# ishine/TTS-3

Hardware: AMD Instinct MI355X
Metric: audio samples/sec + RTF, HiFiGAN-v1 22.05kHz 80-mel, batch 32 @ 1/2/4/8 GPU (higher is better)
Workload: dtype fp32 (power-of-2 scaled fp16 hi/lo split on fp16 MFMA, fp32 accumulate); 1 GPU; HiFiGAN-v1 22.05kHz inference, [32,80,1024] mel per GPU (replicate pad 5), fp32; model=HiFiGAN-v1 (hifigan_config.py generator_model_params), global_batch=32, seq_len=1024, parallelism=dp1 (utterance sharding; no collectives)

## Files before the change

tts-3_amd/csrc/common.hpp:

```cpp
#pragma once

#include <hip/hip_runtime.h>

#include <cstdint>
#include <stdexcept>
#include <string>

namespace tts {

struct Error : std::runtime_error {
  int code;
  Error(int c, const std::string& m) : std::runtime_error(m), code(c) {}
};

#define TTS_HIP_CHECK(expr)                                                               \
  do {                                                                                    \
    hipError_t _e = (expr);                                                               \
    if (_e != hipSuccess)                                                                 \
      throw ::tts::Error(2, std::string(#expr) + " failed: " + hipGetErrorString(_e));    \
  } while (0)

#define TTS_REQUIRE(cond, code, msg)                    \
  do {                                                  \
    if (!(cond)) throw ::tts::Error((code), (msg));     \
  } while (0)

typedef float f32x4 __attribute__((ext_vector_type(4)));
typedef float f32x16 __attribute__((ext_vector_type(16)));

__device__ __forceinline__ float lrelu(float x, float slope) { return x > 0.f ? x : x * slope; }

constexpr int kPlaneXB16 = 1;
constexpr int kPlaneYB16 = 2;

struct Conv1dArgs {
  const float* x;
  const float* w;
  const float* bias;
  const float* res;
  float* y;
  float* z;
  const float* cvec;
  const float* mask;
  int64_t x_bstride;
  int Cin, Cout, Tin, Tout;
  int dil, pad, rep_pad;
  int n_chunks;
  float in_slope, out_slope;
  int zmode;
  float zdiv;
  const unsigned* amax_in;
  unsigned* amax_out;
  int w_exp;
  int ups;
  int64_t o_bstride;
  int64_t cvec_bstride;
  int mask_res;
  int wn_rows;
  int gate;
  int planes;
};

constexpr int kSplitGateTile = 20;
constexpr int kSplitWinoTile = 21;
bool wino_supported(int mode, int Cout, int Cin, int K, int dil);
bool wino_enabled();
void launch_wino(int mode, const Conv1dArgs& a, int B, int K, hipStream_t s);
inline int gate_row_order(int rho, int H) {
  const int j = rho / 128, r = rho % 128;
  return r < 64 ? 64 * j + r : H + 64 * j + (r - 64);
}

struct ResPairArgs {
  Conv1dArgs c1;
  Conv1dArgs c2;
  const float* post_w;
  float post_bias;
  float post_slope;
  float* wav;
};
bool resblock_pair_supported(int mode, int C, int K, int dil);
bool resblock_pair_preferred(int mode, int C, int K, int dil);
bool resblock_pair128(int mode, int C, int K);
void launch_resblock_pair(int mode, const ResPairArgs& a, int B, int K, int C, hipStream_t s);

struct ResBlock3Args {
  const float* x;
  const unsigned* amax_in;
  const float* w[6];
  const float* bias[6];
  int w_exp[6];
  int dil[3];
  float* z;
  int zmode;
  float zdiv;
  unsigned* amax_out;
  int T;
  int planes;
  const float* up_w;
  const float* up_bias;
  int up_w_exp;
  float* up_y;
  unsigned* up_amax;
  const float* zp[2];
  int nzp;
};
bool resblock3_supported(int mode, int C, int K, const int* dil);
bool resblock3_up_supported(int mode, int C, int K, const int* dil);
void launch_resblock3(int mode, const ResBlock3Args& a, int B, int C, int K, hipStream_t s);
bool resblock2_supported(int mode, int C, int K, const int* dil);
bool resblock2_preferred(int mode, int C, int K, const int* dil);
int resblock2_geo64(int mode);
void launch_resblock2(int mode, const ResBlock3Args& a, int B, int C, int K, int geo64, hipStream_t s);

struct ConvTile {
  int BM, BN, TM, TN, CK;
  int PD = 1;
  int WINO = 0;
};

struct ConvTArgs {
  const float* x;
  const float* w;
  const float* bias;
  float* y;
  int Cin, Cout, Tin;
  int n_chunks;
  float in_slope;
  unsigned* amax_out;
  const float* cvec;
};

struct PostArgs {
  const float* z;
  const float* w;
  float bias;
  float* y;
  int Cin, T;
  float in_slope;
  int z_b16;
};

int conv1d_tile_for(int Cout, int K, int Cin, int dil, bool res);
ConvTile conv1d_tile(int idx);
int conv1d_num_tiles();
void launch_conv1d(const Conv1dArgs& a, int B, int K, int tile_idx, hipStream_t s);
int convT_tile_for(int Cout, int U);
ConvTile convT_tile(int idx, int U);
void launch_convT(const ConvTArgs& a, int B, int U, int tile_idx, hipStream_t s);
void launch_conv_post(const PostArgs& a, int B, hipStream_t s);
void launch_mel_window(const float* mel, int B, int C, int T, int pad, int64_t w0, int W, float* out, hipStream_t s);
void launch_cond_vec(const float* g, const float* Wc, const float* bc, float* cvec, int B, int Cc,
                     int C0, hipStream_t s);

constexpr int MATH_FP32 = 0;
constexpr int MATH_FP32_X6 = 1;
constexpr int MATH_FP32_F16X3 = 2;
constexpr int MATH_BF16 = 3;
constexpr int MATH_LAST = MATH_BF16;

ConvTile conv1d_split_tile(int mode, int idx);
int conv1d_split_num_tiles(int mode);
int conv1d_split_tile_for(int mode, int Cout, int K, int Cin, int dil, bool res);
void launch_conv1d_split(int mode, const Conv1dArgs& a, int B, int K, int tile_idx, hipStream_t s);
bool convT_res_supported(int mode, const Conv1dArgs& a);
void launch_convT_res(int mode, const Conv1dArgs& a, int B, hipStream_t s);
void launch_amax(const float* x, int64_t n, int B, unsigned* slots, hipStream_t s, int64_t stride = 0);

inline bool is_split_mode(int mode) { return mode == MATH_FP32_X6 || mode == MATH_FP32_F16X3 || mode == MATH_BF16; }
inline ConvTile conv_tile(int mode, int idx) {
  return is_split_mode(mode) ? conv1d_split_tile(mode, idx) : conv1d_tile(idx);
}
inline int conv_tile_for(int mode, int Cout, int K, int Cin, int dil, bool res) {
  return is_split_mode(mode) ? conv1d_split_tile_for(mode, Cout, K, Cin, dil, res)
                             : conv1d_tile_for(Cout, K, Cin, dil, res);
}
inline int conv_num_tiles(int mode) { return is_split_mode(mode) ? conv1d_split_num_tiles(mode) : conv1d_num_tiles(); }
inline void launch_conv(int mode, const Conv1dArgs& a, int B, int K, int tile, hipStream_t s) {
  if (is_split_mode(mode)) launch_conv1d_split(mode, a, B, K, tile, s);
  else launch_conv1d(a, B, K, tile, s);
}

void pack_conv1d(const float* w, int Cout, int Cin, int K, const ConvTile& t, float* out);
int64_t packed_conv1d_numel(int Cout, int Cin, int K, const ConvTile& t);
void pack_convT(const float* w, int Cin, int Cout, int U, const ConvTile& t, float* out);
int64_t packed_convT_numel(int Cin, int Cout, int U, const ConvTile& t);
__host__ __device__ constexpr int quad_pos(int q) { return q == 1 ? 2 : (q == 2 ? 1 : q); }
int pack_conv1d_split(int mode, const float* w, int Cout, int Cin, int K, const ConvTile& t, float* out,
                      bool quad_perm = true);
int64_t packed_conv1d_split_numel(int mode, int Cout, int Cin, int K, const ConvTile& t);
int pack_convT_split(int mode, const float* w, int Cin, int Cout, int U, const ConvTile& t, float* out);
int pack_conv1d_wino(int mode, const float* w, int Cout, int Cin, int K, const ConvTile& t, float* out);
inline int64_t packed_conv_numel(int mode, int Cout, int Cin, int K, const ConvTile& t) {
  if (t.WINO) return packed_conv1d_split_numel(mode, Cout, Cin, 7 * ((K + 3) / 4), t);
  return is_split_mode(mode) ? packed_conv1d_split_numel(mode, Cout, Cin, K, t) : packed_conv1d_numel(Cout, Cin, K, t);
}
inline int pack_conv(int mode, const float* w, int Cout, int Cin, int K, const ConvTile& t, float* out) {
  if (t.WINO) return pack_conv1d_wino(mode, w, Cout, Cin, K, t, out);
  if (is_split_mode(mode)) return pack_conv1d_split(mode, w, Cout, Cin, K, t, out);
  pack_conv1d(w, Cout, Cin, K, t, out);
  return 0;
}

inline int ceil_div(int a, int b) { return (a + b - 1) / b; }

}
```

tts-3_amd/csrc/hifigan.cpp:

```cpp
#include "hifigan.hpp"

#include <algorithm>
#include <cmath>
#include <cstdlib>
#include <vector>

namespace tts {

namespace {
bool valid_conv_k(int k) { return k == 1 || k == 3 || k == 5 || k == 7 || k == 11; }
}

std::vector<int64_t> hifigan_weight_shapes(const TtsHifiganCfg& c) {
  std::vector<int64_t> n;
  const int C0 = c.upsample_initial_channel;
  n.push_back((int64_t)C0 * c.in_channels * 7);
  n.push_back(C0);
  for (int i = 0; i < c.num_upsamples; ++i) {
    const int ci = C0 >> i, co = C0 >> (i + 1);
    n.push_back((int64_t)ci * co * c.upsample_kernel_sizes[i]);
    n.push_back(co);
  }
  for (int i = 0; i < c.num_upsamples; ++i) {
    const int ch = C0 >> (i + 1);
    for (int j = 0; j < c.num_kernels; ++j) {
      const int k = c.resblock_kernel_sizes[j];
      const int nconv = (c.resblock_type == 1) ? 6 : 2;
      for (int m = 0; m < nconv; ++m) {
        n.push_back((int64_t)ch * ch * k);
        n.push_back(ch);
      }
    }
  }
  const int cl = C0 >> c.num_upsamples;
  n.push_back((int64_t)c.out_channels * cl * 7);
  if (c.conv_post_bias) n.push_back(c.out_channels);
  if (c.cond_channels > 0) {
    n.push_back((int64_t)C0 * c.cond_channels);
    n.push_back(C0);
  }
  if (c.cond_in_each_up_layer) {
    for (int i = 0; i < c.num_upsamples; ++i) {
      n.push_back((int64_t)(C0 >> (i + 1)) * c.cond_channels);
      n.push_back(C0 >> (i + 1));
    }
  }
  return n;
}

void hifigan_validate(const TtsHifiganCfg& c) {
  TTS_REQUIRE(c.in_channels >= 1, 1, "in_channels must be >= 1");
  TTS_REQUIRE(c.out_channels == 1, 3, "only out_channels == 1 is implemented");
  TTS_REQUIRE(c.resblock_type == 1 || c.resblock_type == 2, 1, "resblock_type must be '1' or '2'");
  TTS_REQUIRE(c.num_kernels >= 1 && c.num_kernels <= TTS_MAX_KERNELS, 1, "bad num_kernels");
  TTS_REQUIRE(c.num_upsamples >= 1 && c.num_upsamples <= TTS_MAX_UPSAMPLES, 1, "bad num_upsamples");
  const int need_d = c.resblock_type == 1 ? 3 : 2;
  TTS_REQUIRE(c.num_dilations >= need_d && c.num_dilations <= TTS_MAX_DILATIONS, 1,
              "resblock_dilation_sizes too short for the resblock type");
  for (int j = 0; j < c.num_kernels; ++j) {
    TTS_REQUIRE(valid_conv_k(c.resblock_kernel_sizes[j]), 3,
                "resblock kernel size " + std::to_string(c.resblock_kernel_sizes[j]) +
                    " not implemented (1,3,5,7,11)");
    for (int m = 0; m < need_d; ++m) {
      const int d = c.resblock_dilation_sizes[j][m];
      TTS_REQUIRE(d >= 1 && (c.resblock_kernel_sizes[j] - 1) * d <= 96, 3,
                  "resblock (kernel_size-1)*dilation must be <= 96");
    }
  }
  int C = c.upsample_initial_channel;
  for (int i = 0; i < c.num_upsamples; ++i) {
    const int u = c.upsample_factors[i];
    TTS_REQUIRE(u == 2 || u == 4 || u == 8, 3, "upsample factor must be 2, 4 or 8");
    TTS_REQUIRE(c.upsample_kernel_sizes[i] == 2 * u, 3,
                "upsample kernel size must equal 2*factor (polyphase kernel)");
    C >>= 1;
    TTS_REQUIRE(C >= 1, 1, "upsample_initial_channel too small for the number of upsamples");
  }
  TTS_REQUIRE(c.inference_padding >= 0, 1, "inference_padding must be >= 0");
  TTS_REQUIRE(c.cond_channels >= 0, 1, "cond_channels must be >= 0");
  TTS_REQUIRE(!c.cond_in_each_up_layer || c.cond_channels > 0, 1, "cond_in_each_up_layer needs cond_channels > 0");
  TTS_REQUIRE(c.math_mode >= MATH_FP32 && c.math_mode <= MATH_LAST, 1, "unknown math_mode");
}

Hifigan::Hifigan(const TtsHifiganCfg& cfg, const float* const* hw, int device)
    : cfg_(cfg), device_(device) {
  hifigan_validate(cfg_);
  DeviceGuard g(device_);
  const auto shapes = hifigan_weight_shapes(cfg_);
  for (size_t i = 0; i < shapes.size(); ++i)
    TTS_REQUIRE(hw[i] != nullptr, 1, "weight pointer " + std::to_string(i) + " is NULL");

  const int C0 = cfg_.upsample_initial_channel;
  const int mode = cfg_.math_mode;
  const char* nf = std::getenv("TTS_MI355X_NO_PAIR_FUSION");
  const bool pair_fusion = !(nf && nf[0] == '1');
  const char* pf = std::getenv("TTS_MI355X_POST_FUSION");
  post_fusion_ = !(pf && pf[0] == '0');
  const char* ms = std::getenv("TTS_MI355X_MRF_STREAMS");
  nbs_ = ms ? std::max(1, std::min(std::atoi(ms), cfg.num_kernels)) : cfg.num_kernels;
  nbs_env_ = ms != nullptr;
  const char* sb = std::getenv("TTS_MI355X_SUBBATCH");
  n_lanes_ = sb ? std::max(1, std::min(std::atoi(sb), 8)) : 2;
  rb2_geo64_ = resblock2_geo64(mode);
  const char* bp = std::getenv("TTS_MI355X_BF16_PLANES");
  planes16_ = mode == MATH_BF16 && !(bp && bp[0] == '0') && cfg_.num_upsamples >= 1 &&
              cfg_.upsample_factors[0] % 8 == 0;
  size_t wi = 0;
  std::vector<std::pair<const float*, const float*>> src;
  auto add_conv = [&](int Cin, int Cout, int K, int dil, const char* fam, bool res, int lmode, bool pair128 = false) {
    ConvLayer L;
    L.Cin = Cin; L.Cout = Cout; L.K = K; L.dil = dil; L.pad = dil * (K - 1) / 2;
    L.mode = lmode;
    L.tile = conv_tile_for(lmode, Cout, K, Cin, dil, res);
    if (pair128) {
      L.tile = 7;
      L.name = std::string(fam) + "_k" + std::to_string(K) + "_c" + std::to_string(Cout);
      return L;
    }
    const bool wino_k3 = [] {
      const char* e = std::getenv("TTS_MI355X_WINO_K3");
      return e && e[0] == '1';
    }();
    const bool k_ok = K >= 7 || (K == 3 && Cout >= 256 && wino_k3);
    if (std::string(fam) == "mrf_conv" && k_ok && wino_enabled() && wino_supported(lmode, Cout, Cin, K, dil)) {
      L.tile = kSplitWinoTile;
      fam = "mrf_wino";
    }
    L.name = std::string(fam) + "_k" + std::to_string(K) + "_c" + std::to_string(Cout);
    return L;
  };

  pre_ = add_conv(cfg_.in_channels, C0, 7, 1, "conv_pre", false, mode);
  src.push_back({hw[wi], hw[wi + 1]}); wi += 2;
  for (int i = 0; i < cfg_.num_upsamples; ++i) {
    ConvTLayer L;
    L.Cin = C0 >> i; L.Cout = C0 >> (i + 1); L.U = cfg_.upsample_factors[i];
    L.mode = mode;
    L.tile = is_split_mode(mode) ? conv_tile_for(mode, L.U * L.Cout, 2, L.Cin, 1, false) : convT_tile_for(L.Cout, L.U);
    L.name = "ups_u" + std::to_string(L.U) + "_c" + std::to_string(L.Cout);
    ups_.push_back(L);
  }
  std::vector<std::pair<const float*, const float*>> usrc;
  for (int i = 0; i < cfg_.num_upsamples; ++i) { usrc.push_back({hw[wi], hw[wi + 1]}); wi += 2; }

  for (int i = 0; i < cfg_.num_upsamples; ++i) {
    const int ch = C0 >> (i + 1);
    for (int j = 0; j < cfg_.num_kernels; ++j) {
      const int k = cfg_.resblock_kernel_sizes[j];
      ResBlock rb;
      if (cfg_.resblock_type == 1) {
        const float* w1[3]; const float* b1[3]; const float* w2[3]; const float* b2[3];
        for (int m = 0; m < 3; ++m) { w1[m] = hw[wi]; b1[m] = hw[wi + 1]; wi += 2; }
        for (int m = 0; m < 3; ++m) { w2[m] = hw[wi]; b2[m] = hw[wi + 1]; wi += 2; }
        rb.fused = pair_fusion;
        const bool p128 = pair_fusion && resblock_pair128(mode, ch, k);
        bool tiles_ok = true;
        for (int m = 0; m < 3; ++m) {
          rb.convs.push_back(add_conv(ch, ch, k, cfg_.resblock_dilation_sizes[j][m], "mrf_conv", false, mode, p128));
          src.push_back({w1[m], b1[m]});
          rb.convs.push_back(add_conv(ch, ch, k, 1, "mrf_conv", true, mode, p128));
          src.push_back({w2[m], b2[m]});
          for (int c = 0; c < 2; ++c) {
            const ConvTile t = conv_tile(mode, rb.convs[2 * m + c].tile);
            const int dil = rb.convs[2 * m].dil;
            tiles_ok = tiles_ok && !t.WINO && t.CK % 16 == 0 && ch % t.CK == 0 && ch % t.BM == 0;
            rb.fused = rb.fused && !t.WINO && t.CK == 16 && ceil_div(ch, t.BM) * t.BM == ch &&
                       resblock_pair_preferred(mode, ch, k, dil);
          }
        }
        rb.fused3 = pair_fusion && tiles_ok;
      } else {
        bool tiles_ok = true;
        for (int m = 0; m < 2; ++m) {
          rb.convs.push_back(add_conv(ch, ch, k, cfg_.resblock_dilation_sizes[j][m], "mrf_conv", true, mode));
          src.push_back({hw[wi], hw[wi + 1]}); wi += 2;
          const ConvTile t = conv_tile(mode, rb.convs[m].tile);
          tiles_ok = tiles_ok && !t.WINO && t.CK % 16 == 0 && ch % t.CK == 0 && ch % t.BM == 0;
        }
        rb.fused2 = pair_fusion && tiles_ok;
      }
      if (rb.fused2 || (cfg_.resblock_type == 1 && rb.fused3)) {
        const int policy = [] {
          const char* e = std::getenv("TTS_MI355X_RESBLOCK3");
          if (!e) return 1 << 30;
          if (std::string(e) == "all") return 1 << 30;
          return std::atoi(e);
        }();
        const std::string wk = [] {
          const char* e = std::getenv("TTS_MI355X_RB1_WHOLE_K");
          return std::string(e ? e : "");
        }();
        const bool k_ok = k == 3 || wk.find(std::to_string(k)) != std::string::npos;
        if (cfg_.resblock_type == 1)
          rb.fused3 = ch <= policy && k_ok && resblock3_supported(mode, ch, k, cfg_.resblock_dilation_sizes[j]);
        else
          rb.fused2 = ch <= policy && resblock2_preferred(mode, ch, k, cfg_.resblock_dilation_sizes[j]);
      }
      res_.push_back(rb);
    }
  }
  ups_fused_.assign(cfg_.num_upsamples, 0);
  const char* uf = std::getenv("TTS_MI355X_UPS_FUSION");
  if (!(uf && uf[0] == '0') && cfg_.resblock_type == 1 && cfg_.num_kernels <= 3 && !cfg_.cond_in_each_up_layer &&
      !planes16_) {
    for (int i = 0; i + 1 < cfg_.num_upsamples; ++i) {
      const int ch = C0 >> (i + 1);
      const ConvTLayer& u = ups_[i + 1];
      if (!res_[i * cfg_.num_kernels].fused3 || u.U != 2 || !is_split_mode(u.mode)) continue;
      const ConvTile t = conv_tile(u.mode, u.tile);
      const bool tile_ok = !t.WINO && t.CK % 16 == 0 && ch % t.CK == 0 && ch % t.BM == 0;
      ups_fused_[i] = tile_ok && resblock3_up_supported(mode, ch, cfg_.resblock_kernel_sizes[0],
                                                        cfg_.resblock_dilation_sizes[0]);
    }
  }
  const float* post_w = hw[wi]; wi += 1;
  post_bias_ = cfg_.conv_post_bias ? hw[wi][0] : 0.f;
  if (cfg_.conv_post_bias) wi += 1;

  HostArena arena;
  std::vector<ConvLayer*> convs;
  convs.push_back(&pre_);
  for (auto& rb : res_) for (auto& c : rb.convs) convs.push_back(&c);
  for (size_t i = 0; i < convs.size(); ++i) {
    ConvLayer& c = *convs[i];
    arena.put_conv(c, c.mode, conv_tile(c.mode, c.tile), src[i].first, src[i].second);
  }
  for (size_t i = 0; i < ups_.size(); ++i) {
    auto& u = ups_[i];
    if (is_split_mode(u.mode)) {
      const ConvTile t = conv_tile(u.mode, u.tile);
      u.n_chunks = ceil_div(u.Cin, t.CK);
      const size_t o = arena.alloc(packed_conv_numel(u.mode, u.U * u.Cout, u.Cin, 2, t), &u.w);
      u.w_exp = pack_convT_split(u.mode, usrc[i].first, u.Cin, u.Cout, u.U, t, arena.at(o));
      std::vector<float> bias((size_t)u.U * u.Cout);
      for (int co = 0; co < u.Cout; ++co)
        for (int ph = 0; ph < u.U; ++ph) bias[(size_t)co * u.U + ph] = usrc[i].second[co];
      arena.put_bias(bias.data(), u.U * u.Cout, t, &u.b);
    } else {
      const ConvTile t = convT_tile(u.tile, u.U);
      u.n_chunks = ceil_div(u.Cin, t.CK);
      const size_t o = arena.alloc(packed_convT_numel(u.Cin, u.Cout, u.U, t), &u.w);
      pack_convT(usrc[i].first, u.Cin, u.Cout, u.U, t, arena.at(o));
      arena.put_bias(usrc[i].second, u.Cout, t, &u.b);
    }
  }
  arena.put(post_w, (size_t)(C0 >> cfg_.num_upsamples) * 7, &post_wd_);
  if (cfg_.cond_channels > 0) {
    arena.put(hw[wi], (size_t)C0 * cfg_.cond_channels, &cond_wd_);
    arena.put(hw[wi + 1], C0, &cond_bd_);
    wi += 2;
  }
  if (cfg_.cond_in_each_up_layer) {
    up_cond_.resize(cfg_.num_upsamples);
    for (int i = 0; i < cfg_.num_upsamples; ++i) {
      const size_t ci = C0 >> (i + 1);
      arena.put(hw[wi], ci * cfg_.cond_channels, &up_cond_[i].first);
      arena.put(hw[wi + 1], ci, &up_cond_[i].second);
      wi += 2;
    }
  }
  arena.upload(device_, arena_);
  hop_ = 1;
  for (int i = 0; i < cfg_.num_upsamples; ++i) hop_ *= cfg_.upsample_factors[i];
}

Hifigan::~Hifigan() {
  DeviceGuard g(device_);
  for (Lane& ln : lanes_) {
    for (hipStream_t st : ln.branch) (void)hipStreamDestroy(st);
    if (ln.own) (void)hipStreamDestroy(ln.own);
    for (hipEvent_t e : ln.ev_z) (void)hipEventDestroy(e);
    if (ln.ev_ups) (void)hipEventDestroy(ln.ev_ups);
    if (ln.ev_done) (void)hipEventDestroy(ln.ev_done);
  }
  if (ev_start_) (void)hipEventDestroy(ev_start_);
}

int64_t Hifigan::out_len(int T, int pad) const { return (int64_t)hop_ * (T + 2 * pad); }

int64_t Hifigan::plane_floats(int B, int T, int pad) const {
  const int64_t L = T + 2 * pad;
  int64_t best = (int64_t)cfg_.upsample_initial_channel * L;
  int64_t len = L;
  for (int i = 0; i < cfg_.num_upsamples; ++i) {
    len *= cfg_.upsample_factors[i];
    const int64_t c = (int64_t)(cfg_.upsample_initial_channel >> (i + 1)) * len;
    if (c > best) best = c;
  }
  return ((best * B + 63) / 64) * 64;
}

int Hifigan::n_planes(int nbs) const { return 2 + 2 * nbs; }

int Hifigan::split_nbs() const { return nbs_env_ ? nbs_ : 1; }

void Hifigan::ensure_lanes() {
  if (!lanes_.empty()) return;
  auto stream = [] {
    hipStream_t st;
    TTS_HIP_CHECK(hipStreamCreateWithFlags(&st, hipStreamNonBlocking));
    return st;
  };
  auto event = [] {
    hipEvent_t e;
    TTS_HIP_CHECK(hipEventCreateWithFlags(&e, hipEventDisableTiming));
    return e;
  };
  lanes_.resize(n_lanes_);
  for (int i = 0; i < n_lanes_; ++i) {
    Lane& ln = lanes_[i];
    if (i > 0) ln.own = stream();
    for (int j = 1; j < nbs_; ++j) ln.branch.push_back(stream());
    ln.ev_ups = event();
    ln.ev_done = event();
    for (int j = 0; j < cfg_.num_kernels; ++j) ln.ev_z.push_back(event());
  }
  ev_start_ = event();
}

int64_t Hifigan::lane_bytes(int B, int64_t L, int nbs) const {
  const int64_t cond = cond_floats(B);
  const int64_t amax = cfg_.math_mode == MATH_FP32_F16X3 ? (int64_t)amax_groups() * B * 64 : 0;
  return ((n_planes(nbs) * plane_floats(B, (int)L, 0) + cond + amax + 63) / 64 * 64) * (int64_t)sizeof(float);
}

int Hifigan::amax_groups() const { return 2 + cfg_.num_upsamples * (2 + cfg_.num_kernels * 6); }
int Hifigan::stage_group(int i) const { return 2 + i * (2 + cfg_.num_kernels * 6); }

int64_t Hifigan::cond_floats(int B) const {
  if (cfg_.cond_channels <= 0) return 0;
  int64_t n = (((int64_t)B * cfg_.upsample_initial_channel + 63) / 64) * 64;
  if (cfg_.cond_in_each_up_layer)
    for (int i = 0; i < cfg_.num_upsamples; ++i)
      n += (((int64_t)B * (cfg_.upsample_initial_channel >> (i + 1)) + 63) / 64) * 64;
  return n;
}

int Hifigan::window_halo() const {
  double r = 3.0, rate = 1.0;
  for (int i = 0; i < cfg_.num_upsamples; ++i) {
    r += 1.5 / rate;
    rate *= cfg_.upsample_factors[i];
    int widest = 0;
    for (int j = 0; j < cfg_.num_kernels; ++j) {
      const int h = (cfg_.resblock_kernel_sizes[j] - 1) / 2;
      int w = 0;
      for (int m = 0; m < (cfg_.resblock_type == 1 ? 3 : 2); ++m)
        w += h * cfg_.resblock_dilation_sizes[j][m] + (cfg_.resblock_type == 1 ? h : 0);
      widest = std::max(widest, w);
    }
    r += widest / rate;
  }
  r += 3.0 / rate;
  return (int)std::ceil(r) + 2;
}

int64_t Hifigan::max_window_frames() const {
  int64_t cr = cfg_.upsample_initial_channel, rate = 1;
  for (int i = 0; i < cfg_.num_upsamples; ++i) {
    rate *= cfg_.upsample_factors[i];
    cr = std::max(cr, (int64_t)(cfg_.upsample_initial_channel >> (i + 1)) * rate);
  }
  return ((int64_t(1) << 29) - 1) / cr;
}

int64_t Hifigan::window_payload() const {
  const char* e = std::getenv("TTS_MI355X_WINDOW_FRAMES");
  const int64_t cap = max_window_frames() - 2 * window_halo();
  if (e && std::atoll(e) > 0) return std::min<int64_t>(std::atoll(e), cap);
  return cap;
}

bool Hifigan::windowed(int64_t L) const {
  const char* e = std::getenv("TTS_MI355X_WINDOW_FRAMES");
  return L > max_window_frames() || (e && std::atoll(e) > 0 && L > std::atoll(e));
}

int64_t Hifigan::plain_workspace_bytes(int B, int64_t L, bool window) const {
  const int nl = std::min(n_lanes_, B);
  if (window || nl == 1) return lane_bytes(B, L, nbs_);
  int64_t lanes = 0;
  for (int i = 0; i < nl; ++i) lanes += lane_bytes(lane_batch(B, i), L, split_nbs());
  return std::max(lane_bytes(B, L, 1), lanes);
}

int64_t Hifigan::window_buffer_bytes(int B, int64_t W) const {
  return ((((int64_t)B * cfg_.in_channels * W + 63) / 64) * 64 + (int64_t)B * hop_ * W) * (int64_t)sizeof(float);
}

int64_t Hifigan::workspace_bytes(int B, int T, int pad) const {
  const int64_t L = (int64_t)T + 2 * pad;
  if (!windowed(L)) return plain_workspace_bytes(B, L, false);
  const int64_t W = std::min<int64_t>(L, window_payload() + 2 * window_halo());
  return plain_workspace_bytes(B, W, true) + window_buffer_bytes(B, W);
}

void Hifigan::reserve_plain(int B, int64_t L, bool window) {
  const int64_t need = plain_workspace_bytes(B, L, window);
  ws_.grow(device_, (size_t)need, "workspace");
}

void Hifigan::reserve(int B, int T, int pad) {
  const int64_t L = (int64_t)T + 2 * pad;
  if (!windowed(L)) {
    reserve_plain(B, L);
    return;
  }
  const int64_t W = std::min<int64_t>(L, window_payload() + 2 * window_halo());
  reserve_plain(B, W, true);
  win_.grow(device_, (size_t)window_buffer_bytes(B, W), "window buffers");
}

void Hifigan::forward(const float* mel, int B, int C, int T, int pad, const float* gvec, float* wav,
                      hipStream_t s, Profiler* prof) {
  TTS_REQUIRE(mel && wav, 1, "NULL input/output pointer");
  TTS_REQUIRE(B >= 1, 1, "batch must be >= 1");
  TTS_REQUIRE(C == cfg_.in_channels, 1,
              "mel has " + std::to_string(C) + " channels, generator expects " + std::to_string(cfg_.in_channels));
  TTS_REQUIRE(T >= 1, 1, "T must be >= 1");
  TTS_REQUIRE(pad >= 0, 1, "pad must be >= 0");
  TTS_REQUIRE(cfg_.cond_channels == 0 || gvec != nullptr, 1, "cond_channels > 0 requires g");
  const int64_t L = (int64_t)T + 2 * pad;
  if (!windowed(L)) {
    DeviceGuard dg(device_);
    reserve_plain(B, L);
    if (prof) {
      forward_plain(mel, B, C, T, pad, gvec, wav, s, prof, ws_.as<>(), nullptr);
      return;
    }
    ensure_lanes();
    const int nl = std::min(n_lanes_, B);
    for (Lane& ln : lanes_) ln.nbs = nl > 1 ? split_nbs() : nbs_;
    if (nl == 1) {
      forward_plain(mel, B, C, T, pad, gvec, wav, s, nullptr, ws_.as<>(), &lanes_[0]);
      return;
    }
    TTS_HIP_CHECK(hipEventRecord(ev_start_, s));
    float* ws = ws_.as<>();
    int b0 = 0;
    for (int i = 0; i < nl; ++i) {
      const int Bi = lane_batch(B, i);
      Lane& ln = lanes_[i];
      const hipStream_t si = i == 0 ? s : ln.own;
      if (i > 0) TTS_HIP_CHECK(hipStreamWaitEvent(si, ev_start_, 0));
      forward_plain(mel + (int64_t)b0 * C * T, Bi, C, T, pad,
                    gvec ? gvec + (int64_t)b0 * cfg_.cond_channels : nullptr, wav + (int64_t)b0 * out_len(T, pad), si,
                    nullptr, ws, &ln);
      if (i > 0) {
        TTS_HIP_CHECK(hipEventRecord(ln.ev_done, si));
        TTS_HIP_CHECK(hipStreamWaitEvent(s, ln.ev_done, 0));
      }
      ws += lane_bytes(Bi, L, ln.nbs) / (int64_t)sizeof(float);
      b0 += Bi;
    }
    return;
  }
  DeviceGuard dg(device_);
  reserve(B, T, pad);
  const int h = window_halo();
  const int64_t P = window_payload();
  TTS_REQUIRE(P >= 1, 3, "window payload must be >= 1 frame");
  const int64_t Wmax = std::min<int64_t>(L, P + 2 * h);
  float* melw = win_.as<>();
  float* outw = melw + (((int64_t)B * C * Wmax + 63) / 64) * 64;
  for (int64_t s0 = 0; s0 < L; s0 += P) {
    const int64_t s1 = std::min(L, s0 + P);
    const int64_t w0 = std::max<int64_t>(0, s0 - h), w1 = std::min(L, s1 + h);
    const int W = (int)(w1 - w0);
    run(prof, s, "mel_window", 0.0, 8.0 * B * C * (double)W,
        [&] { launch_mel_window(mel, B, C, T, pad, w0, W, melw, s); });
    if (!prof) {
      ensure_lanes();
      lanes_[0].nbs = nbs_;
    }
    forward_plain(melw, B, C, W, 0, gvec, outw, s, prof, ws_.as<>(), prof ? nullptr : &lanes_[0]);
    TTS_HIP_CHECK(hipMemcpy2DAsync(wav + hop_ * s0, sizeof(float) * hop_ * L, outw + hop_ * (s0 - w0),
                                   sizeof(float) * hop_ * W, sizeof(float) * hop_ * (s1 - s0), B,
                                   hipMemcpyDeviceToDevice, s));
  }
}

void Hifigan::forward_plain(const float* mel, int B, int C, int T, int pad, const float* gvec, float* wav,
                            hipStream_t s, Profiler* prof, float* ws, Lane* lane) {
  DeviceGuard g(device_);

  const int64_t plane = plane_floats(B, T, pad);
  float* bufZ = ws;
  float* bufO = ws + plane;
  float* bufT0 = ws + 3 * plane;
  const int np = n_planes(lane ? lane->nbs : 1);
  float* cvec = cfg_.cond_channels > 0 ? ws + np * plane : nullptr;
  const bool h3 = cfg_.math_mode == MATH_FP32_F16X3;
  unsigned* amax = h3 ? reinterpret_cast<unsigned*>(ws + np * plane + cond_floats(B)) : nullptr;
  const int nbs = lane ? lane->nbs : 1;
  const bool conc = nbs > 1;
  const int K = cfg_.num_kernels;
  auto bstream = [&](int j) { return std::max(0, j - (K - nbs)); };
  auto slots = [&](int grp) -> unsigned* { return amax ? amax + (size_t)grp * B * 64 : nullptr; };
  if (h3) TTS_HIP_CHECK(hipMemsetAsync(amax, 0, (size_t)amax_groups() * B * 64 * sizeof(unsigned), s));

  const int L = T + 2 * pad;
  const int C0 = cfg_.upsample_initial_channel;
  bool post_done = false;
  if (cvec) {
    run(prof, s, "cond_layer", 2.0 * B * C0 * cfg_.cond_channels, 4.0 * (B * cfg_.cond_channels + C0 * cfg_.cond_channels + B * C0),
        [&] { launch_cond_vec(gvec, cond_wd_, cond_bd_, cvec, B, cfg_.cond_channels, C0, s); });
  }

  auto conv = [&](const ConvLayer& Ld, const float* x, int Tin, int Tout, int rep, float in_slope,
                  float out_slope, const float* res, float* y, int zmode, const float* cv,
                  const unsigned* amax_in = nullptr, unsigned* amax_out = nullptr, hipStream_t st = nullptr) {
    if (!st) st = s;
    Conv1dArgs a{};
    a.amax_in = amax_in; a.amax_out = amax_out; a.w_exp = Ld.w_exp;
    a.x = x; a.w = Ld.w; a.bias = Ld.b; a.res = res; a.y = y; a.z = bufZ; a.cvec = cv;
    a.Cin = Ld.Cin; a.Cout = Ld.Cout; a.Tin = Tin; a.Tout = Tout;
    a.dil = Ld.dil; a.pad = Ld.pad; a.rep_pad = rep; a.n_chunks = Ld.n_chunks;
    a.in_slope = in_slope; a.out_slope = out_slope; a.zmode = zmode; a.zdiv = (float)cfg_.num_kernels;
    a.planes = planes16_ ? (x == mel ? kPlaneYB16 : kPlaneXB16 | kPlaneYB16) : 0;
    const double ex = (planes16_ && x != mel) ? 2.0 : 4.0, ey = planes16_ ? 2.0 : 4.0;
    const double flops = 2.0 * B * Ld.Cout * (double)Ld.Cin * Ld.K * Tout;
    double bytes = ex * B * Ld.Cin * Tin + 4.0 * Ld.Cout * Ld.Cin * Ld.K + ey * B * Ld.Cout * Tout;
    if (res) bytes += ey * B * Ld.Cout * (double)Tout;
    if (zmode >= 2) bytes += ey * B * Ld.Cout * (double)Tout;
    run(prof, st, Ld.name.c_str(), flops, bytes, [&] { launch_conv(Ld.mode, a, B, Ld.K, Ld.tile, st); });
  };

  if (h3)
    run(prof, s, "amax_mel", 0.0, 4.0 * B * C * (double)T,
        [&] { launch_amax(mel, (int64_t)C * T, B, slots(0), s); });
  conv(pre_, mel, T, L, pad, 1.f, 1.f, nullptr, bufZ, 0, cvec, slots(0), slots(1));

  int len = L;
  const float* cur = bufZ;
  float* upvec = cvec ? cvec + (((int64_t)B * C0 + 63) / 64) * 64 : nullptr;
  for (int i = 0; i < cfg_.num_upsamples; ++i) {
    const ConvTLayer& U = ups_[i];
    const int g0 = stage_group(i);
    const float* ucv = nullptr;
    if (cfg_.cond_in_each_up_layer) {
      const int ci = U.Cout;
      run(prof, s, "cond_up", 2.0 * B * ci * cfg_.cond_channels, 4.0 * (B * cfg_.cond_channels + ci * cfg_.cond_channels + B * ci),
          [&] { launch_cond_vec(gvec, up_cond_[i].first, up_cond_[i].second, upvec, B, cfg_.cond_channels, ci, s); });
      ucv = upvec;
      upvec += (((int64_t)B * ci + 63) / 64) * 64;
    }
    const unsigned* z_amax = slots(i == 0 ? 1 : stage_group(i - 1) + 1 + cfg_.num_kernels * 6);
    const int lout = len * U.U;
    const double uflops = 2.0 * B * U.Cout * (double)U.Cin * 2 * lout;
    const double es = planes16_ ? 2.0 : 4.0;
    const double ubytes = es * ((double)B * U.Cin * len + (double)B * U.Cout * lout) + 4.0 * U.Cin * U.Cout * 2 * U.U;
    const bool fuse = ups_fused_[i] != 0;
    const bool ups_done = i > 0 && ups_fused_[i - 1] != 0;
    if (ups_done) {
    } else if (is_split_mode(U.mode)) {
      Conv1dArgs a{};
      a.planes = planes16_ ? kPlaneXB16 | kPlaneYB16 : 0;
      a.x = cur; a.w = U.w; a.bias = U.b; a.y = bufO;
      a.Cin = U.Cin; a.Cout = U.U * U.Cout; a.Tin = len; a.Tout = len + 1;
      a.dil = 1; a.pad = 1; a.n_chunks = U.n_chunks;
      a.in_slope = 0.1f; a.out_slope = 1.f; a.zdiv = 1.f;
      a.amax_in = z_amax; a.amax_out = slots(g0); a.w_exp = U.w_exp; a.ups = U.U;
      a.cvec = ucv;
      run(prof, s, U.name.c_str(), uflops, ubytes, [&] { launch_conv(U.mode, a, B, 2, U.tile, s); });
    } else {
      ConvTArgs ta{};
      ta.x = cur; ta.w = U.w; ta.bias = U.b; ta.y = bufO;
      ta.Cin = U.Cin; ta.Cout = U.Cout; ta.Tin = len; ta.n_chunks = U.n_chunks; ta.in_slope = 0.1f;
      ta.cvec = ucv;
      run(prof, s, U.name.c_str(), uflops, ubytes, [&] { launch_convT(ta, B, U.U, U.tile, s); });
    }
    len = lout;
    if (conc) TTS_HIP_CHECK(hipEventRecord(lane->ev_ups, s));
    float* rplane[TTS_MAX_KERNELS] = {};
    for (int jj = 0; jj < K; ++jj) {
      const int j = fuse ? (jj + 1) % K : jj;
      const ResBlock& rb = res_[i * K + j];
      const int bj = conc ? bstream(j) : 0;
      const hipStream_t sj = bj > 0 ? lane->branch[bj - 1] : s;
      float* bufX = ws + (2 + 2 * bj) * plane;
      float* bufT = bj == 0 ? bufT0 : bufX + plane;
      if (bj > 0) TTS_HIP_CHECK(hipStreamWaitEvent(sj, lane->ev_ups, 0));
      float* const xres = (fuse && j + 1 < K && (conc ? bstream(j + 1) : 0) == bj) ? bufZ : bufX;
      rplane[j] = xres;
      auto zorder = [&] {
        if (!fuse && bj > 0 && bstream(j - 1) != bj) TTS_HIP_CHECK(hipStreamWaitEvent(sj, lane->ev_z[j - 1], 0));
      };
      auto zdone = [&] {
        if (conc) TTS_HIP_CHECK(hipEventRecord(lane->ev_z[j], sj));
      };
      const int zlast = fuse ? 0 : ((cfg_.num_kernels == 1 || j == 0) ? 1 : (j == cfg_.num_kernels - 1 ? 3 : 2));
      const int gj = g0 + 1 + j * 6;
      const int gz = g0 + 1 + cfg_.num_kernels * 6;
      if (fuse && j == 0) {
        const ConvTLayer& Un = ups_[i + 1];
        ResBlock3Args ra{};
        ra.x = bufO; ra.amax_in = slots(g0);
        for (int c = 0; c < 6; ++c) { ra.w[c] = rb.convs[c].w; ra.bias[c] = rb.convs[c].b; ra.w_exp[c] = rb.convs[c].w_exp; }
        for (int m = 0; m < 3; ++m) ra.dil[m] = rb.convs[2 * m].dil;
        ra.zdiv = (float)K;
        ra.T = len;
        ra.nzp = K - 1;
        for (int p = 1; p < K; ++p) {
          ra.zp[p - 1] = rplane[p];
          if (conc && bstream(p) > 0) TTS_HIP_CHECK(hipStreamWaitEvent(s, lane->ev_z[p], 0));
        }
        ra.up_w = Un.w; ra.up_bias = Un.b; ra.up_w_exp = Un.w_exp;
        ra.up_y = bufT0; ra.up_amax = slots(stage_group(i + 1));
        const ConvLayer& L1 = rb.convs[0];
        const double flops = 12.0 * B * L1.Cout * (double)L1.Cin * L1.K * len +
                             2.0 * B * Un.Cout * (double)Un.Cin * 2 * (2.0 * len);
        const double bytes = 4.0 * B * L1.Cout * (double)len * (K + 1) + 4.0 * 6.0 * L1.Cout * L1.Cin * L1.K +
                             4.0 * Un.Cin * Un.Cout * 2 * Un.U;
        const std::string nm = "mrf_block_k" + std::to_string(L1.K) + "_c" + std::to_string(L1.Cout);
        run(prof, s, nm.c_str(), flops, bytes, [&] { launch_resblock3(L1.mode, ra, B, L1.Cout, L1.K, s); });
        std::swap(bufO, bufT0);
      } else if (cfg_.resblock_type == 1 && rb.fused3) {
        ResBlock3Args ra{};
        ra.x = bufO; ra.amax_in = slots(g0);
        ra.planes = planes16_ ? kPlaneXB16 | kPlaneYB16 : 0;
        for (int c = 0; c < 6; ++c) { ra.w[c] = rb.convs[c].w; ra.bias[c] = rb.convs[c].b; ra.w_exp[c] = rb.convs[c].w_exp; }
        for (int m = 0; m < 3; ++m) ra.dil[m] = rb.convs[2 * m].dil;
        ra.z = fuse ? xres : bufZ; ra.zmode = fuse ? 1 : zlast; ra.zdiv = (float)cfg_.num_kernels;
        ra.amax_out = !fuse && j == cfg_.num_kernels - 1 ? slots(gz) : nullptr;
        ra.T = len;
        const ConvLayer& L1 = rb.convs[0];
        const double flops = 12.0 * B * L1.Cout * (double)L1.Cin * L1.K * len;
        const double bytes = (planes16_ ? 2.0 : 4.0) * B * L1.Cout * len * (zlast >= 2 ? 3 : 2) +
                             4.0 * 6.0 * L1.Cout * L1.Cin * L1.K;
        const std::string nm = "mrf_block_k" + std::to_string(L1.K) + "_c" + std::to_string(L1.Cout);
        zorder();
        run(prof, sj, nm.c_str(), flops, bytes, [&] { launch_resblock3(L1.mode, ra, B, L1.Cout, L1.K, sj); });
        zdone();
      } else if (cfg_.resblock_type == 1 && rb.fused) {
        for (int m = 0; m < 3; ++m) {
          const ConvLayer& L1 = rb.convs[2 * m];
          const ConvLayer& L2 = rb.convs[2 * m + 1];
          const float* xin = (m == 0) ? bufO : (m == 1 ? bufX : bufT);
          const bool last = (m == 2);
          float* xout = (m == 1) ? bufT : (last ? xres : bufX);
          ResPairArgs pa{};
          Conv1dArgs& c1 = pa.c1;
          c1.x = xin; c1.w = L1.w; c1.bias = L1.b; c1.Cin = L1.Cin; c1.Cout = L1.Cout; c1.Tin = len; c1.Tout = len;
          c1.dil = L1.dil; c1.pad = L1.pad; c1.n_chunks = L1.n_chunks; c1.in_slope = 0.1f; c1.out_slope = 0.1f;
          c1.zdiv = 1.f; c1.w_exp = L1.w_exp;
          c1.planes = planes16_ ? kPlaneXB16 | kPlaneYB16 : 0;
          c1.amax_in = (m == 0) ? slots(g0) : slots(gj + 2 * m - 1);
          Conv1dArgs& c2 = pa.c2;
          c2.x = nullptr; c2.w = L2.w; c2.bias = L2.b; c2.res = xin; c2.y = xout; c2.z = bufZ;
          c2.Cin = L2.Cin; c2.Cout = L2.Cout; c2.Tin = len; c2.Tout = len; c2.dil = 1; c2.pad = L2.pad;
          c2.n_chunks = L2.n_chunks; c2.in_slope = 1.f; c2.out_slope = 1.f; c2.zmode = last ? zlast : 0;
          c2.zdiv = (float)cfg_.num_kernels; c2.w_exp = L2.w_exp;
          c2.planes = c1.planes;
          c2.amax_out = last ? (!fuse && j == cfg_.num_kernels - 1 ? slots(gz) : nullptr) : slots(gj + 2 * m + 1);
          const bool post = last && zlast == 3 && i == cfg_.num_upsamples - 1 && post_fusion_ &&
                            cfg_.out_channels == 1;
          if (post) {
            pa.post_w = post_wd_; pa.post_bias = post_bias_; pa.post_slope = 0.01f; pa.wav = wav;
            c2.amax_out = nullptr;
            post_done = true;
          }
          double flops = 4.0 * B * L1.Cout * (double)L1.Cin * L1.K * len;
          const double es = planes16_ ? 2.0 : 4.0;
          double bytes = es * B * L1.Cout * len * (last ? (zlast >= 2 ? 4 : 3) : 3) + 4.0 * 2.0 * L1.Cout * L1.Cin * L1.K;
          if (post) {
            flops += 2.0 * B * len * (double)L1.Cout * 7;
            bytes += 4.0 * B * len - es * B * L1.Cout * len;
          }
          const std::string nm = std::string(post ? "mrf_pair_post_k" : "mrf_pair_k") + std::to_string(L1.K) +
                                 "_c" + std::to_string(L1.Cout);
          if (last) zorder();
          run(prof, sj, nm.c_str(), flops, bytes, [&] { launch_resblock_pair(L1.mode, pa, B, L1.K, L1.Cout, sj); });
          if (last) zdone();
        }
      } else if (cfg_.resblock_type == 1) {
        for (int m = 0; m < 3; ++m) {
          const float* xin = (m == 0) ? bufO : bufX;
          const unsigned* xin_amax = (m == 0) ? slots(g0) : slots(gj + 2 * m - 1);
          const bool last = (m == 2);
          conv(rb.convs[2 * m], xin, len, len, 0, 0.1f, 0.1f, nullptr, bufT, 0, nullptr, xin_amax, slots(gj + 2 * m),
               sj);
          if (last) zorder();
          conv(rb.convs[2 * m + 1], bufT, len, len, 0, 1.f, 1.f, xin, last ? xres : bufX, last ? zlast : 0, nullptr,
               slots(gj + 2 * m), last ? (!fuse && j == cfg_.num_kernels - 1 ? slots(gz) : nullptr) : slots(gj + 2 * m + 1), sj);
          if (last) zdone();
        }
      } else if (rb.fused2) {
        ResBlock3Args ra{};
        ra.x = bufO; ra.amax_in = slots(g0);
        ra.planes = planes16_ ? kPlaneXB16 | kPlaneYB16 : 0;
        for (int c = 0; c < 2; ++c) {
          ra.w[c] = rb.convs[c].w; ra.bias[c] = rb.convs[c].b; ra.w_exp[c] = rb.convs[c].w_exp;
          ra.dil[c] = rb.convs[c].dil;
        }
        ra.z = bufZ; ra.zmode = zlast; ra.zdiv = (float)cfg_.num_kernels;
        ra.amax_out = j == cfg_.num_kernels - 1 ? slots(gz) : nullptr;
        ra.T = len;
        const ConvLayer& L1 = rb.convs[0];
        const double flops = 4.0 * B * L1.Cout * (double)L1.Cin * L1.K * len;
        const double bytes = (planes16_ ? 2.0 : 4.0) * B * L1.Cout * len * (zlast >= 2 ? 3 : 2) +
                             4.0 * 2.0 * L1.Cout * L1.Cin * L1.K;
        const std::string nm = "mrf_block2_k" + std::to_string(L1.K) + "_c" + std::to_string(L1.Cout);
        zorder();
        run(prof, sj, nm.c_str(), flops, bytes,
            [&] { launch_resblock2(L1.mode, ra, B, L1.Cout, L1.K, rb2_geo64_, sj); });
        zdone();
      } else {
        for (int m = 0; m < 2; ++m) {
          const float* xin = (m == 0) ? bufO : bufX;
          const unsigned* xin_amax = (m == 0) ? slots(g0) : slots(gj + m - 1);
          const bool last = (m == 1);
          if (last) zorder();
          conv(rb.convs[m], xin, len, len, 0, 0.1f, 1.f, xin, bufX, last ? zlast : 0, nullptr, xin_amax,
               last ? (j == cfg_.num_kernels - 1 ? slots(gz) : nullptr) : slots(gj + m), sj);
          if (last) zdone();
        }
      }
    }
    if (!fuse && conc && bstream(K - 1) > 0) TTS_HIP_CHECK(hipStreamWaitEvent(s, lane->ev_z[K - 1], 0));
    cur = bufZ;
  }
  if (post_done) return;
  PostArgs pa{};
  pa.z = bufZ; pa.w = post_wd_; pa.bias = post_bias_; pa.y = wav;
  pa.Cin = C0 >> cfg_.num_upsamples; pa.T = len; pa.in_slope = 0.01f;
  pa.z_b16 = planes16_ ? 1 : 0;
  run(prof, s, "conv_post", 2.0 * B * len * (double)pa.Cin * 7,
      (planes16_ ? 2.0 : 4.0) * B * pa.Cin * len + 4.0 * B * len, [&] { launch_conv_post(pa, B, s); });
}

}
```

tts-3_amd/csrc/hifigan.hpp:

```cpp
#pragma once

#include <string>
#include <vector>

#include "arena.hpp"
#include "common.hpp"
#include "tts_mi355x.h"

namespace tts {

struct Profiler {
  struct Rec {
    std::string name;
    double flops, bytes;
    hipEvent_t a, b;
  };
  std::vector<Rec> recs;
  ~Profiler() {
    for (auto& r : recs) {
      (void)hipEventDestroy(r.a);
      (void)hipEventDestroy(r.b);
    }
  }
};

template <class F>
void run(Profiler* p, hipStream_t s, const char* name, double flops, double bytes, F&& launch) {
  if (!p) {
    launch();
    return;
  }
  Profiler::Rec r{name, flops, bytes, nullptr, nullptr};
  TTS_HIP_CHECK(hipEventCreate(&r.a));
  TTS_HIP_CHECK(hipEventCreate(&r.b));
  TTS_HIP_CHECK(hipEventRecord(r.a, s));
  launch();
  TTS_HIP_CHECK(hipEventRecord(r.b, s));
  p->recs.push_back(r);
}

std::vector<int64_t> hifigan_weight_shapes(const TtsHifiganCfg& c);
void hifigan_validate(const TtsHifiganCfg& c);

class Hifigan {
 public:
  Hifigan(const TtsHifiganCfg& cfg, const float* const* host_weights, int device);
  ~Hifigan();
  Hifigan(const Hifigan&) = delete;
  Hifigan& operator=(const Hifigan&) = delete;

  int64_t out_len(int T, int pad) const;
  int64_t workspace_bytes(int B, int T, int pad) const;
  void reserve(int B, int T, int pad);
  void forward(const float* mel, int B, int C, int T, int pad, const float* g, float* wav,
               hipStream_t s, Profiler* prof);
  int device() const { return device_; }
  int window_halo() const;
  int64_t max_window_frames() const;
  int64_t window_payload() const;

 private:
  struct ConvLayer : PackedConv {
    int mode = 0;
    std::string name;
  };
  struct ConvTLayer : PackedConv {
    int U = 0;
    int mode = 0;
    std::string name;
  };
  struct ResBlock {
    std::vector<ConvLayer> convs;
    bool fused = false;
    bool fused3 = false;
    bool fused2 = false;
  };

  struct Lane {
    hipStream_t own = nullptr;
    std::vector<hipStream_t> branch;
    hipEvent_t ev_ups = nullptr, ev_done = nullptr;
    std::vector<hipEvent_t> ev_z;
    int nbs = 1;
  };
  void forward_plain(const float* mel, int B, int C, int T, int pad, const float* g, float* wav, hipStream_t s,
                     Profiler* prof, float* ws, Lane* lane);
  void ensure_lanes();
  int64_t lane_bytes(int B, int64_t L, int nbs) const;
  int lane_batch(int B, int i) const { return B / n_lanes_ + (i < B % n_lanes_ ? 1 : 0); }
  bool windowed(int64_t L) const;
  int64_t plain_workspace_bytes(int B, int64_t L, bool window) const;
  int64_t window_buffer_bytes(int B, int64_t W) const;
  void reserve_plain(int B, int64_t L, bool window = false);
  int64_t plane_floats(int B, int T, int pad) const;
  int64_t cond_floats(int B) const;
  int amax_groups() const;
  int stage_group(int i) const;
  int n_planes(int nbs) const;
  int split_nbs() const;

  TtsHifiganCfg cfg_;
  int device_;
  int hop_ = 1;
  int rb2_geo64_ = 0;
  bool post_fusion_ = true;
  bool planes16_ = false;
  std::vector<char> ups_fused_;
  int nbs_ = 1;
  int n_lanes_ = 2;
  bool nbs_env_ = false;
  std::vector<Lane> lanes_;
  hipEvent_t ev_start_ = nullptr;
  ConvLayer pre_;
  std::vector<ConvTLayer> ups_;
  std::vector<ResBlock> res_;
  float post_bias_ = 0.f;
  float* post_wd_ = nullptr;
  float* cond_wd_ = nullptr;
  float* cond_bd_ = nullptr;
  std::vector<std::pair<float*, float*>> up_cond_;
  DeviceBuffer arena_, ws_;
  DeviceBuffer win_;
};

}
```

tts-3_amd/csrc/kernels_resblock.hip:

```cpp
#include <algorithm>
#include <cstdlib>
#include <type_traits>

#include "resblock_block.hpp"
#include "split_device.hpp"

namespace tts {




constexpr int kPostK = 7;
constexpr int kPostHalo = 3;

template <class S, int K, int C, int PD, int GEO, bool ALLX = false, bool POST = false>
struct PairCfg {
  static constexpr int RP_W = (GEO == 0 || GEO == 4 || GEO == 5 || GEO == 7) ? 256 : (GEO == 1 ? 192 : 128);
  static constexpr int LEAD = (K - 1) / 2;
  static constexpr int RP_BN = RP_W - 2 * LEAD;
  static constexpr int NW = GEO >= 5 ? 8 : 4;
  static constexpr int NT = 64 * NW;
  static constexpr int WN = (GEO == 0 || GEO == 5) ? 4 : (GEO == 8 ? 1 : 2);
  static constexpr int WM = NW / WN;
  static constexpr int TM = C / 32 / WM;
  static constexpr int TN = RP_W / 32 / WN;
  static constexpr int NC = C / 16;
  static constexpr int HMAX = (K - 1) * 5;
  static constexpr int XROWS = RP_W + HMAX;
  static constexpr int XSZB = XROWS * S::ROWB;
  static constexpr int TROWS = RP_W + 32;
  static constexpr int TSZB = NC * TROWS * S::ROWB;
  static constexpr int XBUFS = ALLX ? NC : 2;
  static constexpr int LDSB0 = (XBUFS * XSZB > TSZB ? XBUFS * XSZB : TSZB);
  static constexpr int ZTB = POST ? C * RP_BN * 4 : 0;
  static constexpr int LDSB = LDSB0 > ZTB ? LDSB0 : ZTB;
  static constexpr int STRIDE = POST ? RP_BN - 2 * kPostHalo : RP_BN;
  static constexpr int UPT = (XROWS * 4 + NT - 1) / NT;
  static_assert(TM >= 1 && TM * WM * 32 == C && TN * WN * 32 == RP_W, "geometry");
};

#ifndef PAIR_W_B1
#define PAIR_W_B1 3
#endif
template <class S, int K, int C, int PD, int GEO, bool ALLX, bool POST = false, int PL = 0>
__global__ __launch_bounds__((PairCfg<S, K, C, PD, GEO, ALLX, POST>::NT)) __attribute__((amdgpu_waves_per_eu(
    C > 64 ? (GEO >= 5 ? 2 : 1) : (S::NP == 1 && PAIR_W_B1 > 0 ? PAIR_W_B1 : ((C == 32 || GEO == 2) && S::ROWB <= 80 ? 3 : 1)))))
void resblock_pair_kernel(ResPairArgs pa) {
  constexpr bool XB = (PL & kPlaneXB16) != 0, YB = (PL & kPlaneYB16) != 0;
  using PX = PlaneT<XB>;
  using PY = PlaneT<YB>;
  using P = PairCfg<S, K, C, PD, GEO, ALLX, POST>;
  constexpr int RP_W = P::RP_W, RP_BN = P::RP_BN;
  constexpr int NP = S::NP;
  constexpr bool H3 = S::SCALED;
  constexpr int TM = P::TM, TN = P::TN, NC = P::NC;
  __shared__ __attribute__((aligned(16))) unsigned char smem[P::LDSB];
  __shared__ float red[P::NW];
  constexpr int NT = P::NT;
  __shared__ float bsm[2 * C];
  __shared__ float pws[POST ? C * kPostK : 1];

  const Conv1dArgs& a1 = pa.c1;
  const int tid = threadIdx.x;
  const float bias1 = tid < C ? a1.bias[tid] : 0.f;
  const float bias2 = tid < C ? pa.c2.bias[tid] : 0.f;
  const int lane = tid & 63;
  const int wave = tid >> 6;
  const int half = lane >> 5;
  const int l32 = lane & 31;
  const int wm = __builtin_amdgcn_readfirstlane(wave / P::WN);
  const int wn = wave % P::WN;
  const int mrow0 = wm * TM * 32;
  const int t0 = (int)blockIdx.x * P::STRIDE - (POST ? kPostHalo : 0);
  const int b = blockIdx.z;
  const int d = a1.dil;
  const int T = a1.Tout;
  const int XW = RP_W + (K - 1) * d;
  const int tx0 = t0 - P::LEAD;
  const unsigned avoff = (unsigned)lane * 16u;

  auto post_epilogue = [&](const ResPairArgs& q, const f32x16 (&ac)[TM][TN], int bb, int tt0, int row0w, int wnn,
                           int ln) {
    const Conv1dArgs a2 = q.c2;
    const int hf = ln >> 5, lo = ln & 31;
    const size_t item = (size_t)bb * C * T;
    const unsigned plane = (unsigned)C * (unsigned)T * PY::ES;
    const rsrc_t rres = make_rsrc(plane_at<YB>(a2.res, item), plane);
    const rsrc_t rz = make_rsrc(plane_at<YB>(a2.z, item), plane);
    const unsigned rowb = (unsigned)T * PY::ES;
    float* zt = reinterpret_cast<float*>(smem);
    __syncthreads();
#pragma unroll
    for (int m = 0; m < TM; ++m) {
#pragma unroll
      for (int n = 0; n < TN; ++n) {
        const int col = wnn * TN * 32 + n * 32 + lo;
        const int t = tt0 + col;
        const bool tok = t >= 0 && t < T && col < RP_BN;
        const int rw0 = row0w + m * 32 + 4 * hf;
        const unsigned voff = tok ? ((unsigned)rw0 * (unsigned)T + (unsigned)t) * PY::ES : OOB_OFF;
        float rv[16], zv[16];
#pragma unroll
        for (int r = 0; r < 16; ++r) {
          const unsigned vo = voff + (unsigned)((r & 3) + 8 * (r >> 2)) * rowb;
          rv[r] = PY::ld(rres, vo, 0u);
          zv[r] = PY::ld(rz, vo, 0u);
        }
        if (col < RP_BN) {
#pragma unroll
          for (int r = 0; r < 16; ++r) {
            const int row = rw0 + (r & 3) + 8 * (r >> 2);
            float v = (ac[m][n][r] + bsm[C + row]) * 1.f;
            v = lrelu2(v, a2.out_slope);
            v = (v + rv[r]) * 1.f;
            v = (zv[r] + v) / a2.zdiv;
            zt[row * RP_BN + col] = tok ? lrelu(PY::rt(v), q.post_slope) : 0.f;
          }
        }
      }
    }
    __syncthreads();
    const int col = kPostHalo + tid;
    const int t = tt0 + col;
    if (col < RP_BN - kPostHalo && t >= 0 && t < T) {
      float o = q.post_bias;
#pragma unroll 4
      for (int ci = 0; ci < C; ++ci) {
        const float* zr = zt + ci * RP_BN + col - kPostHalo;
#pragma unroll
        for (int k = 0; k < kPostK; ++k) o = fmaf(pws[ci * kPostK + k], zr[k], o);
      }
      q.wav[(size_t)bb * T + t] = tanhf(o);
    }
  };

  const int ex = H3 ? amax_exp(a1.amax_in, b) : 0;
  const float xscale = H3 ? ldexpf(1.f, -ex) : 1.f;
  const char* xb = static_cast<const char*>(plane_at<XB>(a1.x, (size_t)b * C * T));
  const unsigned chb = (unsigned)T * PX::ES;
  unsigned uvoff[P::UPT];
  int ulds[P::UPT];
#pragma unroll
  for (int i = 0; i < P::UPT; ++i) {
    const int u = tid + i * NT;
    const int q = RES_STAGE_8R ? quad_pos((u >> 3) & 3) : (u & 3);
    const int r = RES_STAGE_8R ? (u >> 5) * 8 + (u & 7) : (u >> 2);
    const int ts = tx0 - a1.pad + r;
    const bool ok = r < XW && ts >= 0 && ts < T;
    uvoff[i] = ok ? (unsigned)(4 * q) * chb + (unsigned)ts * PX::ES : OOB_OFF;
    ulds[i] = r < XW ? r * S::ROWB + 8 * quad_pos(q) : -1;
  }
  f32x4 xall[ALLX ? NC : 1][P::UPT];
  auto load_x = [&](int c) {
    f32x4 (&xreg)[P::UPT] = xall[ALLX ? c : 0];
    const rsrc_t rx = make_rsrc(xb + (size_t)c * 16 * chb, (unsigned)(C - c * 16) * chb);
#pragma unroll
    for (int i = 0; i < P::UPT; ++i)
#pragma unroll
      for (int j = 0; j < 4; ++j) xreg[i][j] = PX::ld(rx, uvoff[i] + (unsigned)j * chb, 0u);
  };
  auto store_x = [&](int buf, int c) {
    const f32x4 (&xreg)[P::UPT] = xall[ALLX ? c : 0];
    unsigned char* xl = smem + buf * P::XSZB;
#pragma unroll
    for (int i = 0; i < P::UPT; ++i) {
      if (ulds[i] >= 0) {
        float v[4];
#pragma unroll
        for (int j = 0; j < 4; ++j) {
          v[j] = lrelu2(xreg[i][j], a1.in_slope);
          if (H3) v[j] *= xscale;
        }
        split_store4<S>(xl + ulds[i], v[0], v[1], v[2], v[3]);
      }
    }
  };

  rsrc_t ra[TM];
#pragma unroll
  for (int m = 0; m < TM; ++m) ra[m] = make_rsrc(a1.w + ((size_t)(wm * TM + m) * NC * K) * (NP * 256), 0xFFFFFFFFu);

  f32x16 acc[TM][TN];
#pragma unroll
  for (int m = 0; m < TM; ++m)
#pragma unroll
    for (int n = 0; n < TN; ++n) acc[m][n] = f32x16{};

  f32x4 ar[PD + 1][TM][NP], bcur[TN][NP], bnext[TN][NP];
#pragma unroll
  for (int p = 0; p < PD; ++p)
#pragma unroll
    for (int m = 0; m < TM; ++m)
#pragma unroll
      for (int q = 0; q < NP; ++q) ar[p][m][q] = bload4(ra[m], avoff, (unsigned)(p * NP + q) * 1024u);

  auto mfma_step = [&]() {
#pragma unroll
    for (int e = 0; e < S::NPROD; ++e)
#pragma unroll
      for (int m = 0; m < TM; ++m)
#pragma unroll
        for (int n = 0; n < TN; ++n)
          acc[m][n] = S::mfma(ar[0][m][S::PA[e]], bcur[n][S::PB[e]], acc[m][n]);
#pragma unroll
    for (int p = 0; p < PD; ++p)
#pragma unroll
      for (int m = 0; m < TM; ++m)
#pragma unroll
        for (int q = 0; q < NP; ++q) ar[p][m][q] = ar[p + 1][m][q];
  };

  const int xrow0 = wn * TN * 32 + l32;
  auto read_x = [&](const unsigned char* xl, int k, f32x4 (*dst)[NP]) {
#pragma unroll
    for (int n = 0; n < TN; ++n) {
      const unsigned char* p = xl + (xrow0 + n * 32 + k * d) * S::ROWB + 16 * half;
#pragma unroll
      for (int q = 0; q < NP; ++q) dst[n][q] = *reinterpret_cast<const f32x4*>(p + 32 * q);
    }
  };

  if constexpr (ALLX) {
#pragma unroll
    for (int c = 0; c < NC; ++c) load_x(c);
#pragma unroll
    for (int c = 0; c < NC; ++c) store_x(c, c);
  } else {
    load_x(0);
    store_x(0, 0);
  }
  if (tid < C) {
    bsm[tid] = bias1;
    bsm[C + tid] = bias2;
  }
  if constexpr (POST)
    for (int e = tid; e < C * kPostK; e += NT) pws[e] = pa.post_w[e];
  __syncthreads();
#pragma unroll
  for (int c = 0; c < NC; ++c) {
    const unsigned char* xl = smem + (ALLX ? c : (c & 1)) * P::XSZB;
    if (!ALLX && c + 1 < NC) load_x(c + 1);
    read_x(xl, 0, bcur);
#pragma unroll
    for (int k = 0; k < K; ++k) {
      const int s = c * K + k;
#pragma unroll
      for (int m = 0; m < TM; ++m)
#pragma unroll
        for (int q = 0; q < NP; ++q) ar[PD][m][q] = bload4(ra[m], avoff, (unsigned)((s + PD) * NP + q) * 1024u);
      if (k + 1 < K) read_x(xl, k + 1, bnext);
      __builtin_amdgcn_sched_barrier(0);
      mfma_step();
      if (k + 1 < K) {
#pragma unroll
        for (int n = 0; n < TN; ++n)
#pragma unroll
          for (int q = 0; q < NP; ++q) bcur[n][q] = bnext[n][q];
      }
    }
    if (!ALLX && c + 1 < NC) store_x((c + 1) & 1, c + 1);
    if (!ALLX || c + 1 == NC) __syncthreads();
  }

  {
    const float sc1 = H3 ? ldexpf(1.f, ex + a1.w_exp) : 1.f;
    float tmax = 0.f;
#pragma unroll
    for (int m = 0; m < TM; ++m) {
      float bv[16];
#pragma unroll
      for (int r = 0; r < 16; ++r) bv[r] = bsm[mrow0 + m * 32 + (r & 3) + 8 * (r >> 2) + 4 * half];
#pragma unroll
      for (int n = 0; n < TN; ++n) {
        const int t = tx0 + xrow0 + n * 32;
        const bool inside = t >= 0 && t < T;
#pragma unroll
        for (int r = 0; r < 16; ++r) {
          float v = lrelu2(acc[m][n][r] * sc1 + bv[r], a1.out_slope);
          v = inside ? v : 0.f;
          acc[m][n][r] = v;
          tmax = fmaxf(tmax, fabsf(v));
        }
      }
    }
    float tscale = 1.f;
    int et = 0;
    if (H3) {
      tmax = wave_max(tmax);
      if (lane == 0) red[wave] = tmax;
      __syncthreads();
      float mx = red[0];
#pragma unroll
      for (int w = 1; w < P::NW; ++w) mx = fmaxf(mx, red[w]);
      if (mx > 0.f && mx < INFINITY) {
        int E;
        (void)frexpf(mx, &E);
        et = E - 14;
      }
      tscale = ldexpf(1.f, -et);
    }
#pragma unroll
    for (int m = 0; m < TM; ++m)
#pragma unroll
      for (int n = 0; n < TN; ++n)
#pragma unroll
        for (int gl = 0; gl < 2; ++gl)
          store_xt8<S>(smem + (((mrow0 + m * 32) / 16 + gl) * P::TROWS + xrow0 + n * 32) * S::ROWB + 16 * half,
                       acc[m][n], 8 * gl, tscale);
    constexpr int ZB = (P::TROWS - RP_W) * S::ROWB;
    for (int e = tid * 16; e < NC * ZB; e += NT * 16) {
      const int g = e / ZB;
      *reinterpret_cast<f32x4*>(smem + (g * P::TROWS + RP_W) * S::ROWB + (e - g * ZB)) = f32x4{};
    }
    __syncthreads();
    const Conv1dArgs& a2 = pa.c2;
#pragma unroll
    for (int m = 0; m < TM; ++m) ra[m] = make_rsrc(a2.w + ((size_t)(wm * TM + m) * NC * K) * (NP * 256), 0xFFFFFFFFu);
#pragma unroll
    for (int m = 0; m < TM; ++m)
#pragma unroll
      for (int n = 0; n < TN; ++n) acc[m][n] = f32x16{};
#pragma unroll
    for (int p = 0; p < PD; ++p)
#pragma unroll
      for (int m = 0; m < TM; ++m)
#pragma unroll
        for (int q = 0; q < NP; ++q) ar[p][m][q] = bload4(ra[m], avoff, (unsigned)(p * NP + q) * 1024u);
    const int trow0 = xrow0;
    auto read_t = [&](int g, int k, f32x4 (*dst)[NP]) {
#pragma unroll
      for (int n = 0; n < TN; ++n) {
        const unsigned char* p = smem + (g * P::TROWS + trow0 + n * 32 + k) * S::ROWB + 16 * half;
#pragma unroll
        for (int q = 0; q < NP; ++q) dst[n][q] = *reinterpret_cast<const f32x4*>(p + 32 * q);
      }
    };
    read_t(0, 0, bcur);
#pragma unroll
    for (int g = 0; g < NC; ++g) {
#pragma unroll
      for (int k = 0; k < K; ++k) {
        const int s = g * K + k;
#pragma unroll
        for (int m = 0; m < TM; ++m)
#pragma unroll
          for (int q = 0; q < NP; ++q) ar[PD][m][q] = bload4(ra[m], avoff, (unsigned)((s + PD) * NP + q) * 1024u);
        const bool more = (k + 1 < K) || (g + 1 < NC);
        if (more) read_t((k + 1 < K) ? g : g + 1, (k + 1 < K) ? k + 1 : 0, bnext);
        __builtin_amdgcn_sched_barrier(0);
        mfma_step();
        if (more) {
#pragma unroll
          for (int n = 0; n < TN; ++n)
#pragma unroll
            for (int q = 0; q < NP; ++q) bcur[n][q] = bnext[n][q];
        }
      }
    }
    if (H3) {
      const float sc2 = ldexpf(1.f, et + a2.w_exp);
#pragma unroll
      for (int m = 0; m < TM; ++m)
#pragma unroll
        for (int n = 0; n < TN; ++n) acc[m][n] *= sc2;
    }
    if constexpr (POST) {
      post_epilogue(pa, acc, b, t0, mrow0, wn, lane);
    } else {
      conv_epilogue<TM, TN, H3, YB>(a2, acc, b, t0 + wn * TN * 32, mrow0, lane, t0 + RP_BN, bsm + C);
    }
  }
}

namespace {
template <class S, int K, int C, int GEO>
void launch_pair_t(const ResPairArgs& a, int B, hipStream_t s) {
  constexpr bool AX = C == 64 && GEO != 2;
  constexpr int PD = S::NP == 1 ? RES_PD_B1 : 2;
  auto go = [&](auto pl_tag) {
    constexpr int PL = decltype(pl_tag)::value;
    if (a.post_w) {
      using P = PairCfg<S, K, C, PD, GEO, AX, true>;
      static_assert(P::RP_BN - 2 * kPostHalo <= 256, "one conv_post column per thread");
      dim3 grid(ceil_div(a.c1.Tout, P::STRIDE), 1, B);
      hipLaunchKernelGGL((resblock_pair_kernel<S, K, C, PD, GEO, AX, true, PL>), grid, dim3(P::NT), 0, s, a);
      return;
    }
    using P = PairCfg<S, K, C, PD, GEO, AX>;
    dim3 grid(ceil_div(a.c1.Tout, P::RP_BN), 1, B);
    hipLaunchKernelGGL((resblock_pair_kernel<S, K, C, PD, GEO, AX, false, PL>), grid, dim3(P::NT), 0, s, a);
  };
  if (a.c1.planes != 0) {
    constexpr bool OK = std::is_same<S, SchemeB1>::value;
    TTS_REQUIRE(OK && a.c1.planes == (kPlaneXB16 | kPlaneYB16) && a.c2.planes == a.c1.planes, 3,
                "resblock pair: bf16 planes need the bf16 scheme");
    if constexpr (OK) go(std::integral_constant<int, kPlaneXB16 | kPlaneYB16>{});
    return;
  }
  go(std::integral_constant<int, 0>{});
}

int pair_geo64() {
  static const int g = [] {
    const char* e = std::getenv("TTS_MI355X_PAIR_GEO64");
    return e && std::atoi(e) == 2 ? 2 : (e && std::atoi(e) == 4 ? 4 : 1);
  }();
  return g;
}

template <class S, int K>
void launch_pair_k(const ResPairArgs& a, int B, int C, hipStream_t s) {
  if constexpr (S::NP == 1) {
    if (C == 128) {
      static const int geo = [] {
        const char* e = std::getenv("TTS_MI355X_PAIR128_GEO");
        return e && e[0] == '2' ? 2 : (e && e[0] == '0' ? 0 : (e && e[0] == '4' ? 4 : (e && e[0] == '5' ? 5 : 7)));
      }();
      if (geo == 2) launch_pair_t<S, K, 128, 2>(a, B, s);
      else if (geo == 7) launch_pair_t<S, K, 128, 7>(a, B, s);
      else if (geo == 5) launch_pair_t<S, K, 128, 5>(a, B, s);
      else if (geo == 4) launch_pair_t<S, K, 128, 4>(a, B, s);
      else launch_pair_t<S, K, 128, 0>(a, B, s);
      return;
    }
    if (C == 256) {
      static const int geo = [] {
        const char* e = std::getenv("TTS_MI355X_PAIR256_GEO");
        return e && e[0] == '2' ? 2 : (e && e[0] == '6' ? 6 : 8);
      }();
      if (geo == 6) launch_pair_t<S, K, 256, 6>(a, B, s);
      else if (geo == 8) launch_pair_t<S, K, 256, 8>(a, B, s);
      else launch_pair_t<S, K, 256, 2>(a, B, s);
      return;
    }
  }
  if (C == 32) launch_pair_t<S, K, 32, 0>(a, B, s);
  else if (C == 64 && pair_geo64() == 2 && S::ROWB <= 80) launch_pair_t<S, K, 64, 2>(a, B, s);
  else if (C == 64 && pair_geo64() == 4 && S::NP == 1) launch_pair_t<S, K, 64, 4>(a, B, s);
  else if (C == 64) launch_pair_t<S, K, 64, 1>(a, B, s);
  else throw Error(3, "resblock pair: channels must be 32 or 64");
}

template <class S>
void launch_pair_s(const ResPairArgs& a, int B, int K, int C, hipStream_t s) {
  switch (K) {
    case 3: launch_pair_k<S, 3>(a, B, C, s); break;
    case 7: launch_pair_k<S, 7>(a, B, C, s); break;
    case 11: launch_pair_k<S, 11>(a, B, C, s); break;
    default: throw Error(3, "resblock pair: kernel size must be 3, 7 or 11");
  }
}
}

bool resblock_pair_supported(int mode, int C, int K, int dil) {
  return is_split_mode(mode) && (C == 32 || C == 64 || ((C == 128 || C == 256) && mode == MATH_BF16)) &&
         (K == 3 || K == 7 || K == 11) && dil >= 1 && dil <= 5;
}

bool resblock_pair128(int mode, int C, int K) {
  if (mode != MATH_BF16) return false;
  const char* e128 = std::getenv("TTS_MI355X_PAIR128");
  const char* e256 = std::getenv("TTS_MI355X_PAIR256");
  if (C == 128) return (K == 7 || K == 11) && !(e128 && e128[0] == '0');
  if (C == 256) {
    const char* e11 = std::getenv("TTS_MI355X_PAIR256_K11");
    return (K == 3 || K == 7 || (K == 11 && e11 && e11[0] == '1')) && !(e256 && e256[0] == '0');
  }
  return false;
}

bool resblock_pair_preferred(int mode, int C, int K, int dil) {
  return resblock_pair_supported(mode, C, K, dil);
}

void launch_resblock_pair(int mode, const ResPairArgs& a, int B, int K, int C, hipStream_t s) {
  TTS_REQUIRE(resblock_pair_supported(mode, C, K, a.c1.dil), 3, "resblock pair: unsupported configuration");
  TTS_REQUIRE(a.c1.Cin == C && a.c1.Cout == C && a.c2.Cin == C && a.c2.Cout == C && a.c1.Tin == a.c1.Tout &&
                  a.c2.Tout == a.c1.Tout && a.c1.rep_pad == 0 && a.c2.dil == 1,
              1, "resblock pair: bad arguments");
  TTS_REQUIRE(a.c2.res != a.c2.y || a.c2.zmode != 0, 1, "resblock pair: x and x' must not alias");
  TTS_REQUIRE(a.c1.cvec == nullptr && a.c2.cvec == nullptr && a.c1.bias && a.c2.bias, 1,
              "resblock pair: biases required, no cond vector (both are staged in LDS)");
  TTS_REQUIRE((int64_t)C * a.c1.Tout * 4 < (int64_t(1) << 31), 3, "resblock pair: plane exceeds 2 GiB");
  TTS_REQUIRE(!a.post_w || (a.c2.zmode == 3 && a.c2.res && a.c2.z && a.wav && !a.c2.mask), 1,
              "resblock pair: the fused conv_post needs the final MRF sum (zmode 3) with a residual");
  if (mode == MATH_FP32_F16X3) launch_pair_s<SchemeH3>(a, B, K, C, s);
  else if (mode == MATH_BF16) launch_pair_s<SchemeB1>(a, B, K, C, s);
  else launch_pair_s<SchemeX6>(a, B, K, C, s);
  TTS_HIP_CHECK(hipGetLastError());
}


namespace {
template <class S, int C, int GEO, int K>
void launch_res3_t(const ResBlock3Args& a, int B, hipStream_t s) {
  using P = Res3Cfg<S, C, GEO, K, 6, r3_xoff(K), r3_lead(K)>;
  dim3 grid(ceil_div(a.T, P::RP_BN), 1, B);
  launch_block_pl<S, C, GEO, K, 6, r3_xoff(K), r3_lead(K)>(a, grid, P::NT, s);
}
template <class S, int C, int GEO>
void launch_res3_up_t(const ResBlock3Args& a, int B, hipStream_t s) {
  using P = Res3Cfg<S, C, GEO, 3, 6, r3_xoff(3), r3_lead(3), true>;
  dim3 grid(ceil_div(a.T, P::RP_BN), 1, B);
  hipLaunchKernelGGL((resblock3_kernel<S, C, GEO, 3, 6, r3_xoff(3), r3_lead(3), 0, true>), grid, dim3(P::NT), 0, s, a);
}
template <class S>
void launch_res3_s(const ResBlock3Args& a, int B, int C, int K, hipStream_t s) {
  if (K == 7) {
    if (C == 32) launch_res3_t<S, 32, 0, 7>(a, B, s);
    else launch_res3_t<S, 64, 0, 7>(a, B, s);
    return;
  }
  if (K == 11) {
    if (C == 32) launch_res3_t<S, 32, 0, 11>(a, B, s);
    else launch_res3_t<S, 64, 0, 11>(a, B, s);
    return;
  }
  if (C == 32) launch_res3_t<S, 32, 0, 3>(a, B, s);
  else if (C == 128) {
    if constexpr (S::NP == 2) launch_res3_t<S, 128, 4, 3>(a, B, s);
    else if constexpr (S::ROWB <= 80) launch_res3_t<S, 128, 3, 3>(a, B, s);
    else throw Error(3, "resblock3: 128 channels need a split scheme of at most 80-byte rows");
  } else launch_res3_t<S, 64, 2, 3>(a, B, s);
}
}

bool resblock3_supported(int mode, int C, int K, const int* dil) {
  if (!is_split_mode(mode)) return false;
  if (K == 3) {
    if (!(C == 32 || C == 64 || (C == 128 && mode != MATH_FP32_X6))) return false;
  } else if (K == 7 || K == 11) {
    if (!(C == 32 || C == 64)) return false;
  } else {
    return false;
  }
  const int hk = (K - 1) / 2;
  int lo = -r3_xoff(K);
  for (int m = 0; m < 3; ++m) {
    if (dil[m] < 1 || hk * dil[m] > r3_xoff(K)) return false;
    lo = std::max(lo + hk * dil[m], 0) + hk;
  }
  return lo <= r3_lead(K);
}

bool resblock3_up_supported(int mode, int C, int K, const int* dil) {
  if (mode != MATH_FP32_F16X3 || K != 3 || !(C == 64 || C == 128) || !resblock3_supported(mode, C, K, dil)) return false;
  const int rp_w = 128;
  int lo = -r3_xoff(K), hi = rp_w + r3_xoff(K);
  for (int m = 0; m < 3; ++m) {
    lo = std::max(lo + dil[m], 0) + 1;
    hi = std::min(hi - dil[m], rp_w) - 1;
  }
  return lo <= r3_lead(K) - 1 && hi >= rp_w - r3_lead(K) + 1;
}

void launch_resblock3(int mode, const ResBlock3Args& a, int B, int C, int K, hipStream_t s) {
  TTS_REQUIRE(resblock3_supported(mode, C, K, a.dil), 3, "resblock3: unsupported configuration");
  TTS_REQUIRE((int64_t)C * a.T * 4 < (int64_t(1) << 31), 3, "resblock3: plane exceeds 2 GiB");
  if (a.up_w) {
    TTS_REQUIRE(resblock3_up_supported(mode, C, K, a.dil), 3, "resblock3: no upsampling tail for this configuration");
    TTS_REQUIRE(a.x && a.up_y && a.up_y != a.x && a.up_bias && a.planes == 0 && a.nzp >= 0 && a.nzp <= 2, 1,
                "resblock3: bad arguments of the upsampling tail");
    for (int p = 0; p < a.nzp; ++p)
      TTS_REQUIRE(a.zp[p] && a.zp[p] != a.up_y, 1, "resblock3: a branch plane is missing or aliases the tail's output");
    if (C == 128) launch_res3_up_t<SchemeH3, 128, 4>(a, B, s);
    else launch_res3_up_t<SchemeH3, 64, 2>(a, B, s);
    TTS_HIP_CHECK(hipGetLastError());
    return;
  }
  TTS_REQUIRE(a.zmode >= 1 && a.zmode <= 3 && a.z && a.x && a.x != a.z, 1, "resblock3: bad arguments");
  if (mode == MATH_FP32_F16X3) launch_res3_s<SchemeH3>(a, B, C, K, s);
  else if (mode == MATH_BF16) launch_res3_s<SchemeB1>(a, B, C, K, s);
  else launch_res3_s<SchemeX6>(a, B, C, K, s);
  TTS_HIP_CHECK(hipGetLastError());
}

bool resblock2_supported(int mode, int C, int K, const int* dil) {
  if (!is_split_mode(mode) || !(K == 3 || K == 5 || K == 7 || K == 11)) return false;
  if (!(C == 32 || C == 64 || (C == 128 && mode != MATH_FP32_X6 && (K == 3 || K == 5)))) return false;
  const int H = rb2_halo(K), hk = (K - 1) / 2;
  int lo = -H;
  for (int m = 0; m < 2; ++m) {
    if (dil[m] < 1 || hk * dil[m] > H) return false;
    lo = std::max(lo + hk * dil[m], 0);
  }
  return lo <= H;
}

bool resblock2_preferred(int mode, int C, int K, const int* dil) {
  if (!resblock2_supported(mode, C, K, dil)) return false;
  const char* e = std::getenv("TTS_MI355X_RB2_ALL");
  if (e && e[0] == '1') return true;
  return mode == MATH_BF16 || !(C == 64 && K == 11);
}

int resblock2_geo64(int mode) {
  const char* e = std::getenv("TTS_MI355X_RB2_GEO64");
  if (e && (e[0] == '0' || e[0] == '1')) return e[0] - '0';
  return mode == MATH_BF16 ? 1 : 0;
}

void launch_resblock2(int mode, const ResBlock3Args& a, int B, int C, int K, int geo64, hipStream_t s) {
  TTS_REQUIRE(resblock2_supported(mode, C, K, a.dil), 3, "resblock2: unsupported configuration");
  TTS_REQUIRE(a.zmode >= 1 && a.zmode <= 3 && a.z && a.x && a.x != a.z, 1, "resblock2: bad arguments");
  TTS_REQUIRE((int64_t)C * a.T * 4 < (int64_t(1) << 31), 3, "resblock2: plane exceeds 2 GiB");
  if (mode == MATH_FP32_F16X3) launch_resblock2_h3(a, B, C, K, geo64, s);
  else if (mode == MATH_BF16) launch_resblock2_b1(a, B, C, K, geo64, s);
  else launch_resblock2_x6(a, B, C, K, geo64, s);
  TTS_HIP_CHECK(hipGetLastError());
}

}
```

tts-3_amd/csrc/resblock_block.hpp:

```cpp
#pragma once
#include <type_traits>

#include "res3_layout.hpp"
#include "split_device.hpp"

#ifndef RES_PD_B1
#define RES_PD_B1 2
#endif
#ifndef RES_STAGE_8R
#define RES_STAGE_8R 1
#endif

namespace tts {

#ifndef R3_XR_POL
#define R3_XR_POL 0
#endif
constexpr int R3_XOFF = 5;
constexpr int R3_LEAD = 12;
constexpr int r3_xoff(int K) { return R3_XOFF * ((K - 1) / 2); }
constexpr int r3_lead(int K) { return R3_LEAD * ((K - 1) / 2); }
constexpr int rb2_halo(int K) { return K == 3 ? 4 : (K == 5 ? 12 : (K == 7 ? 9 : 15)); }

template <class S, int C, int GEO, int K = 3, int NCV = 6, int XO = R3_XOFF, int LEAD = R3_LEAD, bool UP = false>
struct Res3Cfg {
  static constexpr int RP_W = GEO == 0 ? 256 : (GEO == 1 ? 192 : 128);
  static constexpr int RP_BN = RP_W - 2 * LEAD;
  static constexpr int NW = GEO == 3 ? 8 : 4;
  static constexpr int NT = 64 * NW;
  static constexpr int WN = GEO == 0 ? 4 : 2;
  static constexpr int WM = NW / WN;
  static constexpr int TM = C / 32 / WM;
  static constexpr int TN = RP_W / 32 / WN;
  static constexpr int NC = C / 16;
  static constexpr int PR = RP_W + 2 * XO;
  using ROWS = Res3Rows<S::NP, GEO == 4 && S::NP == 2>;
  static_assert(GEO == 4 || ROWS::PITCH == S::ROWB, "the padded layout is the scheme's own row");
  static constexpr int LDSB = NC * PR * ROWS::PITCH;
  static constexpr int LDS_TOTAL = LDSB + 2 * NW * 4 + (NCV + UP) * C * 4;
  static_assert(GEO != 4 || LDS_TOTAL <= 80 * 1024, "GEO 4: two workgroups per CU");
  static_assert(TM >= 1 && TM * WM * 32 == C && TN * WN * 32 == RP_W, "geometry");
};

#ifndef RB3_W_B1
#define RB3_W_B1 0
#endif
#ifndef RB3_W64
#define RB3_W64 2
#endif
template <class S, int C, int GEO, int K, int NCV, int XO, int LEAD, int PL = 0, bool UP = false>
__global__ __launch_bounds__((Res3Cfg<S, C, GEO, K, NCV, XO, LEAD>::NT))
__attribute__((amdgpu_waves_per_eu(S::NP == 1 && RB3_W_B1 > 0 ? RB3_W_B1
                                                                : (C == 64 && GEO == 2 ? RB3_W64 : (C == 32 || GEO >= 3 ? 2 : 1)))))
void resblock3_kernel(ResBlock3Args a) {
  constexpr bool XB = (PL & kPlaneXB16) != 0, YB = (PL & kPlaneYB16) != 0;
  using PX = PlaneT<XB>;
  using PY = PlaneT<YB>;
  using P = Res3Cfg<S, C, GEO, K, NCV, XO, LEAD, UP>;
  using ROWS = typename P::ROWS;
  static_assert(NCV == 6 || NCV == 2, "ResBlock1 (6 convs) or ResBlock2 (2 convs)");
  static_assert(!UP || (NCV == 6 && S::SCALED && PL == 0), "the upsampling tail: ResBlock1, f16x3, fp32 planes");
  constexpr int NP = S::NP;
  constexpr bool H3 = S::SCALED;
  constexpr int TM = P::TM, TN = P::TN, NC = P::NC, PR = P::PR, RP_W = P::RP_W;
  constexpr int PD = S::NP == 1 ? RES_PD_B1 : 2;
  __shared__ __attribute__((aligned(16))) unsigned char smem[P::LDSB];
  constexpr int NT = P::NT;
  __shared__ float red[2][P::NW];
  __shared__ float bsm[(NCV + UP) * C];

  const int tid = threadIdx.x;
  const int lane = tid & 63;
  const int wave = tid >> 6;
  const int half = lane >> 5;
  const int l32 = lane & 31;
  const int wm = __builtin_amdgcn_readfirstlane(wave / P::WN);
  const int wn = wave % P::WN;
  const int mrow0 = wm * TM * 32;
  const int t0 = blockIdx.x * P::RP_BN;
  const int b = blockIdx.z;
  const int T = a.T;
  const int tx0 = t0 - LEAD;
  const int xcol0 = wn * TN * 32 + l32;
  const unsigned avoff = (unsigned)lane * 16u;
  const unsigned chb = (unsigned)T * PX::ES;
  const rsrc_t rx = make_rsrc(plane_at<XB>(a.x, (size_t)b * C * T), (unsigned)C * chb);
  auto ldx = [&](unsigned off, auto pol_tag, unsigned soff = 0u) -> float {
    if constexpr (XB) return PX::ld(rx, off, soff);
    else return bload_x<decltype(pol_tag)::value>(rx, off, soff);
  };
  constexpr bool SOFF = GEO == 4;

  int ex = H3 ? amax_exp(a.amax_in, b) : 0;
  f32x16 xr[TM][TN];
  {
    const float xs = H3 ? ldexpf(1.f, -ex) : 1.f;
    constexpr int UG = (PR * 4 + NT - 1) / NT;
    constexpr int BPT = (C + NT - 1) / NT;
    float bl[NCV][BPT];
#pragma unroll
    for (int i = 0; i < NCV; ++i)
#pragma unroll
      for (int j = 0; j < BPT; ++j) {
        const int e = tid + j * NT;
        bl[i][j] = e < C ? a.bias[i][e] : 0.f;
      }
    float blu[BPT];
#pragma unroll
    for (int j = 0; j < BPT; ++j) {
      const int e = tid + j * NT;
      blu[j] = UP && e < C ? a.up_bias[e] : 0.f;
    }
    f32x4 xv[NC][UG];
#pragma unroll
    for (int g = 0; g < NC; ++g)
#pragma unroll
      for (int i = 0; i < UG; ++i) {
        const int u = tid + i * NT;
        const int q = RES_STAGE_8R ? quad_pos((u >> 3) & 3) : (u & 3);
        const int r = RES_STAGE_8R ? (u >> 5) * 8 + (u & 7) : (u >> 2);
        const int ts = tx0 - XO + r;
        const bool ok = r < PR && ts >= 0 && ts < T;
        const unsigned vo = (unsigned)(16 * g + 4 * q) * chb + (unsigned)ts * PX::ES;
#pragma unroll
        for (int j = 0; j < 4; ++j)
          xv[g][i][j] = ldx(ok ? vo + (unsigned)j * chb : OOB_OFF, std::integral_constant<int, TTS_LDX_POL>{});
      }
    auto load_xr = [&] {
#pragma unroll
      for (int m = 0; m < TM; ++m)
#pragma unroll
        for (int n = 0; n < TN; ++n) {
          const int t = tx0 + xcol0 + n * 32;
          const bool tok = t >= 0 && t < T;
          const unsigned vlane = tok ? (unsigned)(4 * half) * chb + (unsigned)t * PX::ES : OOB_OFF;
#pragma unroll
          for (int r = 0; r < 16; ++r) {
            const int co = mrow0 + m * 32 + (r & 3) + 8 * (r >> 2) + 4 * half;
            if constexpr (SOFF)
              xr[m][n][r] = ldx(vlane, std::integral_constant<int, R3_XR_POL>{}, (unsigned)(co - 4 * half) * chb);
            else
              xr[m][n][r] = ldx(tok ? (unsigned)co * chb + (unsigned)t * PX::ES : OOB_OFF,
                                std::integral_constant<int, R3_XR_POL>{});
          }
        }
    };
#pragma unroll
    for (int g = 0; g < NC; ++g)
#pragma unroll
      for (int i = 0; i < UG; ++i) {
        const int u = tid + i * NT;
        const int q = RES_STAGE_8R ? quad_pos((u >> 3) & 3) : (u & 3);
        const int r = RES_STAGE_8R ? (u >> 5) * 8 + (u & 7) : (u >> 2);
        if (r < PR) {
          float v[4];
#pragma unroll
          for (int j = 0; j < 4; ++j) {
            v[j] = lrelu2(xv[g][i][j], 0.1f);
            if (H3) v[j] *= xs;
          }
          const int qp = quad_pos(q);
          unsigned char* dst[NP];
#pragma unroll
          for (int p = 0; p < NP; ++p) dst[p] = smem + ROWS::off(g * PR + r, (qp >> 1) + 2 * p) + 8 * (qp & 1);
          split_store4<S>(dst, v[0], v[1], v[2], v[3]);
        }
      }
    __builtin_amdgcn_sched_barrier(0);
    load_xr();
#pragma unroll
    for (int i = 0; i < NCV; ++i)
#pragma unroll
      for (int j = 0; j < BPT; ++j) {
        const int e = tid + j * NT;
        if (e < C) bsm[i * C + e] = bl[i][j];
      }
    if constexpr (UP) {
#pragma unroll
      for (int j = 0; j < BPT; ++j) {
        const int e = tid + j * NT;
        if (e < C) bsm[NCV * C + e] = blu[j];
      }
    }
  }
  __syncthreads();

  f32x16 acc[TM][TN];
  f32x4 ar[PD + 1][TM][NP], bcur[TN][NP], bnext[TN][NP];
  rsrc_t ra[TM];
  auto conv_k = [&](const float* wp, int roff, int kstep, auto ktag) __attribute__((always_inline)) {
    constexpr int KT = decltype(ktag)::value;
    if constexpr (ROWS::SWIZZLED) asm volatile("" : "+s"(roff), "+s"(kstep));
#pragma unroll
    for (int m = 0; m < TM; ++m) ra[m] = make_rsrc(wp + ((size_t)(wm * TM + m) * NC * KT) * (NP * 256), 0xFFFFFFFFu);
#pragma unroll
    for (int m = 0; m < TM; ++m)
#pragma unroll
      for (int n = 0; n < TN; ++n) acc[m][n] = f32x16{};
#pragma unroll
    for (int p = 0; p < PD; ++p)
#pragma unroll
      for (int m = 0; m < TM; ++m)
#pragma unroll
        for (int q = 0; q < NP; ++q) ar[p][m][q] = bload4(ra[m], avoff, (unsigned)(p * NP + q) * 1024u);
    auto read_b = [&](int g, int k, f32x4 (*dst)[NP]) __attribute__((always_inline)) {
#pragma unroll
      for (int n = 0; n < TN; ++n) {
        const int o = ROWS::off(g * PR + xcol0 + roff + k * kstep, half);
#pragma unroll
        for (int q = 0; q < NP; ++q)
          dst[n][q] = *reinterpret_cast<const f32x4*>(smem + ROWS::piece(o, q) + n * 32 * ROWS::PITCH);
      }
    };
    read_b(0, 0, bcur);
#pragma unroll
    for (int g = 0; g < NC; ++g) {
#pragma unroll
      for (int k = 0; k < KT; ++k) {
        const int st = g * KT + k;
#pragma unroll
        for (int m = 0; m < TM; ++m)
#pragma unroll
          for (int q = 0; q < NP; ++q)
            ar[PD][m][q] = bload4(ra[m], avoff, (unsigned)((st + PD) * NP + q) * 1024u);
        const bool more = (k + 1 < KT) || (g + 1 < NC);
        if (more) read_b((k + 1 < KT) ? g : g + 1, (k + 1 < KT) ? k + 1 : 0, bnext);
        __builtin_amdgcn_sched_barrier(0);
#pragma unroll
        for (int e = 0; e < S::NPROD; ++e)
#pragma unroll
          for (int m = 0; m < TM; ++m)
#pragma unroll
            for (int n = 0; n < TN; ++n)
              acc[m][n] = S::mfma(ar[0][m][S::PA[e]], bcur[n][S::PB[e]], acc[m][n]);
#pragma unroll
        for (int p = 0; p < PD; ++p)
#pragma unroll
          for (int m = 0; m < TM; ++m)
#pragma unroll
            for (int q = 0; q < NP; ++q) ar[p][m][q] = ar[p + 1][m][q];
        if (more) {
#pragma unroll
          for (int n = 0; n < TN; ++n)
#pragma unroll
            for (int q = 0; q < NP; ++q) bcur[n][q] = bnext[n][q];
        }
      }
    }
  };
  auto conv = [&](int wi, int roff, int kstep) __attribute__((always_inline)) {
    conv_k(a.w[wi], roff, kstep, std::integral_constant<int, K>{});
  };
  int red_half = 0;
  auto tile_exp = [&](float vmax) __attribute__((always_inline)) -> int {
    if (!H3) return 0;
    vmax = wave_max(vmax);
    if (lane == 0) red[red_half][wave] = vmax;
    __syncthreads();
    float mx = red[red_half][0];
#pragma unroll
    for (int w = 1; w < P::NW; ++w) mx = fmaxf(mx, red[red_half][w]);
    red_half ^= 1;
    int e = 0;
    if (mx > 0.f && mx < INFINITY) {
      int E;
      (void)frexpf(mx, &E);
      e = E - 14;
    }
    return e;
  };

  auto store_pieces = [&](int roff, float scale) __attribute__((always_inline)) {
    if constexpr (ROWS::SWIZZLED) asm volatile("" : "+s"(roff));
#pragma unroll
    for (int m = 0; m < TM; ++m)
#pragma unroll
      for (int n = 0; n < TN; ++n)
#pragma unroll
        for (int gl = 0; gl < 2; ++gl) {
          const int o = ROWS::off(((mrow0 + m * 32) / 16 + gl) * PR + xcol0 + roff, half);
          unsigned char* dst[NP];
#pragma unroll
          for (int p = 0; p < NP; ++p) dst[p] = smem + ROWS::piece(o, p) + n * 32 * ROWS::PITCH;
          store_xt8<S>(dst, acc[m][n], 8 * gl, scale);
        }
    constexpr int ROWB = ROWS::PITCH;
    constexpr int EB = 2 * XO * ROWB;
    for (int e = tid * 16; e < NC * EB; e += NT * 16) {
      const int g = e / EB;
      const int o = e - g * EB;
      const int lead_b = roff * ROWB;
      const int tail_b = (PR - roff - RP_W) * ROWB;
      if (o < lead_b) *reinterpret_cast<f32x4*>(smem + g * PR * ROWB + o) = f32x4{};
      else if (o - lead_b < tail_b)
        *reinterpret_cast<f32x4*>(smem + (g * PR + roff + RP_W) * ROWB + (o - lead_b)) = f32x4{};
    }
  };

  constexpr int HK = (K - 1) / 2;
  int lo = -XO, hi = RP_W + XO;
  auto residual_to_lds = [&](int ci) __attribute__((always_inline)) {
    const float sc = H3 ? ldexpf(1.f, ex + a.w_exp[ci]) : 1.f;
    const float* bs = bsm + ci * C;
    float vmax = 0.f;
#pragma unroll
    for (int m = 0; m < TM; ++m) {
      float bv[16];
#pragma unroll
      for (int r = 0; r < 16; ++r) bv[r] = bs[mrow0 + m * 32 + (r & 3) + 8 * (r >> 2) + 4 * half];
#pragma unroll
      for (int n = 0; n < TN; ++n) {
        const int col = xcol0 + n * 32;
        const int t = tx0 + col;
        const bool ok = col >= lo && col < hi && t >= 0 && t < T;
#pragma unroll
        for (int r = 0; r < 16; ++r) {
          const float x1 = (acc[m][n][r] * sc + bv[r]) + xr[m][n][r];
          xr[m][n][r] = x1;
          const float v = ok ? lrelu2(x1, 0.1f) : 0.f;
          acc[m][n][r] = v;
          vmax = fmaxf(vmax, fabsf(v));
        }
      }
    }
    const int e2 = tile_exp(vmax);
    if (!H3) __syncthreads();
    store_pieces(XO, H3 ? ldexpf(1.f, -e2) : 1.f);
    __syncthreads();
    ex = e2;
  };
  auto final_to_z = [&](int ci) __attribute__((always_inline)) {
    const float sc = H3 ? ldexpf(1.f, ex + a.w_exp[ci]) : 1.f;
    const float* bs = bsm + ci * C;
    const unsigned chbz = (unsigned)T * PY::ES;
    const rsrc_t rz = make_rsrc(plane_at<YB>(a.z, (size_t)b * C * T), (unsigned)C * chbz);
    float vmax = 0.f;
#pragma unroll
    for (int m = 0; m < TM; ++m) {
      float bv[16];
#pragma unroll
      for (int r = 0; r < 16; ++r) bv[r] = bs[mrow0 + m * 32 + (r & 3) + 8 * (r >> 2) + 4 * half];
#pragma unroll
      for (int n = 0; n < TN; ++n) {
        const int col = xcol0 + n * 32;
        const int t = tx0 + col;
        const bool keep = col >= LEAD && col < LEAD + P::RP_BN && t >= 0 && t < T;
        unsigned vo[16], so[16];
        float zv[16];
#pragma unroll
        for (int r = 0; r < 16; ++r) {
          const int co = mrow0 + m * 32 + (r & 3) + 8 * (r >> 2) + 4 * half;
          if constexpr (SOFF) {
            vo[r] = keep ? (unsigned)(4 * half) * chbz + (unsigned)t * PY::ES : OOB_OFF;
            so[r] = (unsigned)(co - 4 * half) * chbz;
          } else {
            vo[r] = keep ? (unsigned)co * chbz + (unsigned)t * PY::ES : OOB_OFF;
            so[r] = 0u;
          }
          zv[r] = a.zmode >= 2 ? PY::ld(rz, vo[r], so[r]) : 0.f;
        }
#pragma unroll
        for (int r = 0; r < 16; ++r) {
          float v = (acc[m][n][r] * sc + bv[r]) + xr[m][n][r];
          if (a.zmode == 2) v = zv[r] + v;
          else if (a.zmode == 3) v = (zv[r] + v) / a.zdiv;
          if (keep) vmax = fmaxf(vmax, fabsf(v));
          PY::st(rz, v, vo[r], so[r]);
        }
      }
    }
    if (H3 && a.amax_out) publish_amax(a.amax_out, b, vmax);
  };

  auto final_up = [&](int ci) __attribute__((always_inline)) {
    const float sc = ldexpf(1.f, ex + a.w_exp[ci]);
    const float* bs = bsm + ci * C;
    const int nzp = a.nzp;
    const float zdiv = a.zdiv;
    rsrc_t rp[2];
#pragma unroll
    for (int p = 0; p < 2; ++p)
      rp[p] = make_rsrc(p < nzp ? a.zp[p] + (size_t)b * C * T : a.x, p < nzp ? (unsigned)C * chb : 0u);
    float vmax = 0.f;
#pragma unroll
    for (int m = 0; m < TM; ++m) {
      float bv[16];
#pragma unroll
      for (int r = 0; r < 16; ++r) bv[r] = bs[mrow0 + m * 32 + (r & 3) + 8 * (r >> 2) + 4 * half];
#pragma unroll
      for (int n = 0; n < TN; ++n) {
        const int col = xcol0 + n * 32;
        const int t = tx0 + col;
        const bool tok = t >= 0 && t < T;
        const unsigned vlane = tok ? (unsigned)(4 * half) * chb + (unsigned)t * 4u : OOB_OFF;
        __builtin_amdgcn_sched_barrier(0);
        float pv[2][16];
#pragma unroll
        for (int p = 0; p < 2; ++p)
#pragma unroll
          for (int r = 0; r < 16; ++r)
            pv[p][r] = bload(rp[p], vlane, (unsigned)(mrow0 + m * 32 + (r & 3) + 8 * (r >> 2)) * chb);
#pragma unroll
        for (int r = 0; r < 16; ++r) {
          float v = (acc[m][n][r] * sc + bv[r]) + xr[m][n][r];
          if (nzp >= 1) v = v + pv[0][r];
          if (nzp >= 2) v = v + pv[1][r];
          asm volatile("" : "+v"(v));
          xr[m][n][r] = v;
        }
      }
    }
    __builtin_amdgcn_sched_barrier(0);
#pragma unroll
    for (int m = 0; m < TM; ++m)
#pragma unroll
      for (int n = 0; n < TN; ++n) {
        const int col = xcol0 + n * 32;
        const int t = tx0 + col;
        const bool ok = col >= lo && col < hi && t >= 0 && t < T;
        __builtin_amdgcn_sched_barrier(0);
#pragma unroll
        for (int r = 0; r < 16; ++r) {
          float v = xr[m][n][r];
          if (nzp >= 1) v = v / zdiv;
          v = ok ? lrelu2(v, 0.1f) : 0.f;
          acc[m][n][r] = v;
          vmax = fmaxf(vmax, fabsf(v));
        }
      }
    const int e2 = tile_exp(vmax);
    store_pieces(XO, ldexpf(1.f, -e2));
    __syncthreads();
    ex = e2;
    conv_k(a.up_w, XO - 1, 1, std::integral_constant<int, 2>{});
    const float sc2 = ldexpf(1.f, ex + a.up_w_exp);
    const float* bu = bsm + NCV * C;
    const int To = 2 * T;
    const unsigned chby = (unsigned)To * 4u;
    const rsrc_t ry = make_rsrc(a.up_y + (size_t)b * (C / 2) * To, (unsigned)(C / 2) * chby);
    const bool last_wg = blockIdx.x == gridDim.x - 1;
    float umax = 0.f;
#pragma unroll
    for (int m = 0; m < TM; ++m) {
      float bv[16];
#pragma unroll
      for (int r = 0; r < 16; ++r) bv[r] = bu[mrow0 + m * 32 + (r & 3) + 8 * (r >> 2) + 4 * half];
#pragma unroll
      for (int n = 0; n < TN; ++n) {
        const int col = xcol0 + n * 32;
        const int mm = tx0 + col;
        const bool keep = col >= LEAD && mm <= T && (col < LEAD + P::RP_BN || (mm == T && last_wg));
        const int ts = 2 * mm - 1;
        const unsigned vl = (unsigned)(2 * half) * chby + (unsigned)ts * 4u;
#pragma unroll
        for (int r = 0; r < 16; r += 2) {
          const unsigned so = (unsigned)((mrow0 + m * 32) / 2 + ((r & 3) >> 1) + 4 * (r >> 2)) * chby;
          const float v0 = acc[m][n][r] * sc2 + bv[r];
          const float v1 = acc[m][n][r + 1] * sc2 + bv[r + 1];
          if (keep && ts >= 0 && ts + 1 < To) {
            umax = fmaxf(umax, fmaxf(fabsf(v0), fabsf(v1)));
            const f32x2 v = {v0, v1};
            __builtin_amdgcn_raw_buffer_store_b64(__builtin_bit_cast(u32x2_t, v), ry, (int)vl, (int)so, TTS_ST_POL);
          } else {
            const bool k0 = keep && ts >= 0, k1 = keep && ts + 1 < To;
            if (k0) umax = fmaxf(umax, fabsf(v0));
            if (k1) umax = fmaxf(umax, fabsf(v1));
            bstore(ry, v0, k0 ? vl : OOB_OFF, so);
            bstore(ry, v1, k1 ? vl + 4u : OOB_OFF, so);
          }
        }
      }
    }
    if (a.up_amax) publish_amax(a.up_amax, b, umax);
  };

  if constexpr (NCV == 6) {
    auto iteration = [&](int it, auto last_tag) __attribute__((always_inline)) {
      constexpr int LAST = decltype(last_tag)::value;
      const int d = a.dil[it];
      conv(2 * it, XO - HK * d, d);
      lo = max(lo + HK * d, 0);
      hi = min(hi - HK * d, RP_W);
      {
        const float sc = H3 ? ldexpf(1.f, ex + a.w_exp[2 * it]) : 1.f;
        const float* bs = bsm + (2 * it) * C;
        float vmax = 0.f;
#pragma unroll
        for (int m = 0; m < TM; ++m) {
          float bv[16];
#pragma unroll
          for (int r = 0; r < 16; ++r) bv[r] = bs[mrow0 + m * 32 + (r & 3) + 8 * (r >> 2) + 4 * half];
#pragma unroll
          for (int n = 0; n < TN; ++n) {
            const int col = xcol0 + n * 32;
            const int t = tx0 + col;
            const bool ok = col >= lo && col < hi && t >= 0 && t < T;
#pragma unroll
            for (int r = 0; r < 16; ++r) {
              float v = lrelu2(acc[m][n][r] * sc + bv[r], 0.1f);
              v = ok ? v : 0.f;
              acc[m][n][r] = v;
              vmax = fmaxf(vmax, fabsf(v));
            }
          }
        }
        const int et = tile_exp(vmax);
        if (!H3) __syncthreads();
        store_pieces(HK, H3 ? ldexpf(1.f, -et) : 1.f);
        __syncthreads();
        ex = et;
      }
      conv(2 * it + 1, 0, 1);
      lo += HK;
      hi -= HK;
      if (LAST == 1 || (LAST == 0 && it < 2)) residual_to_lds(2 * it + 1);
      else if constexpr (UP) final_up(2 * it + 1);
      else final_to_z(2 * it + 1);
    };
    if constexpr (GEO == 4 || UP) {
#pragma unroll 1
      for (int it = 0; it < 2; ++it) iteration(it, std::integral_constant<int, 1>{});
      iteration(2, std::integral_constant<int, 2>{});
    } else {
#pragma unroll 1
      for (int it = 0; it < 3; ++it) iteration(it, std::integral_constant<int, 0>{});
    }
  } else {
#pragma unroll 1
    for (int it = 0; it < 2; ++it) {
      const int d = a.dil[it];
      conv(it, XO - HK * d, d);
      lo = max(lo + HK * d, 0);
      hi = min(hi - HK * d, RP_W);
      if (it == 0) residual_to_lds(0);
      else final_to_z(1);
    }
  }
}

}

namespace tts {
template <class S, int C, int GEO, int K, int NCV, int XO, int LEAD>
void launch_block_pl(const ResBlock3Args& a, dim3 grid, int nt, hipStream_t s) {
  if (a.planes != 0) {
    constexpr bool OK = std::is_same<S, SchemeB1>::value;
    TTS_REQUIRE(OK && a.planes == (kPlaneXB16 | kPlaneYB16), 3, "resblock block: bf16 planes need the bf16 scheme");
    if constexpr (OK)
      hipLaunchKernelGGL((resblock3_kernel<S, C, GEO, K, NCV, XO, LEAD, kPlaneXB16 | kPlaneYB16>), grid, dim3(nt), 0, s, a);
    return;
  }
  hipLaunchKernelGGL((resblock3_kernel<S, C, GEO, K, NCV, XO, LEAD>), grid, dim3(nt), 0, s, a);
}
template <class S, int C, int GEO, int K>
void launch_rb2_t(const ResBlock3Args& a, int B, hipStream_t s) {
  constexpr int H = rb2_halo(K);
  using P = Res3Cfg<S, C, GEO, K, 2, H, H>;
  dim3 grid(ceil_div(a.T, P::RP_BN), 1, B);
  launch_block_pl<S, C, GEO, K, 2, H, H>(a, grid, P::NT, s);
}
template <class S, int C, int GEO>
void launch_rb2_k(const ResBlock3Args& a, int B, int K, hipStream_t s) {
  if (K == 3) launch_rb2_t<S, C, GEO, 3>(a, B, s);
  else if (K == 5) launch_rb2_t<S, C, GEO, 5>(a, B, s);
  else if (K == 7) launch_rb2_t<S, C, GEO, 7>(a, B, s);
  else launch_rb2_t<S, C, GEO, 11>(a, B, s);
}
template <class S>
void launch_rb2_s(const ResBlock3Args& a, int B, int C, int K, int geo64, hipStream_t s) {
  if (C == 32) launch_rb2_k<S, 32, 0>(a, B, K, s);
  else if (C == 64) {
    if (geo64 == 1) launch_rb2_k<S, 64, 1>(a, B, K, s);
    else launch_rb2_k<S, 64, 2>(a, B, K, s);
  } else {
    if constexpr (S::ROWB <= 80) {
      if (K == 3) launch_rb2_t<S, 128, 3, 3>(a, B, s);
      else launch_rb2_t<S, 128, 3, 5>(a, B, s);
    } else {
      throw Error(3, "resblock2: 128 channels need a split scheme of at most 80-byte rows");
    }
  }
}
void launch_resblock2_h3(const ResBlock3Args& a, int B, int C, int K, int geo64, hipStream_t s);
void launch_resblock2_b1(const ResBlock3Args& a, int B, int C, int K, int geo64, hipStream_t s);
void launch_resblock2_x6(const ResBlock3Args& a, int B, int C, int K, int geo64, hipStream_t s);
}
```

Baseline: 170.1 million samples/s.

## Add swizzled 64-byte LDS rows and wide 256-column geometry for C=64 MRF kernels

Introduces a swizzled two-piece LDS row layout (Res3Rows with SWZ) for the 64-channel resblock pair and fused resblock3 kernels in the fp16x3 split mode. These kernels now use a wider 256-column tile with two workgroups per CU. The swizzle targets the 4-way ds_read_b128 bank conflicts that plain 64-byte rows produce, and the wider tile cuts halo overhead per column. In exchange it adds register and LDS pressure and more template instantiations. It is on by default and can be disabled with TTS_MI355X_GEO64_WIDE=0, and a host-side checker replays the LDS addressing to confirm conflict freedom.

```diff
diff --git a/tts-3_amd/csrc/common.hpp b/tts-3_amd/csrc/common.hpp
--- a/tts-3_amd/csrc/common.hpp
+++ b/tts-3_amd/csrc/common.hpp
@@ -82,7 +82,7 @@
 bool resblock_pair_supported(int mode, int C, int K, int dil);
 bool resblock_pair_preferred(int mode, int C, int K, int dil);
 bool resblock_pair128(int mode, int C, int K);
-void launch_resblock_pair(int mode, const ResPairArgs& a, int B, int K, int C, hipStream_t s);
+void launch_resblock_pair(int mode, const ResPairArgs& a, int B, int K, int C, int wide64, hipStream_t s);
 
 struct ResBlock3Args {
   const float* x;
@@ -106,8 +106,10 @@
   int nzp;
 };
 bool resblock3_supported(int mode, int C, int K, const int* dil);
-bool resblock3_up_supported(int mode, int C, int K, const int* dil);
-void launch_resblock3(int mode, const ResBlock3Args& a, int B, int C, int K, hipStream_t s);
+bool resblock3_up_supported(int mode, int C, int K, const int* dil, int wide64);
+constexpr int kWide64Block = 1, kWide64Pair = 2;
+void launch_resblock3(int mode, const ResBlock3Args& a, int B, int C, int K, int wide64, hipStream_t s);
+int mrf_geo64_wide(int mode);
 bool resblock2_supported(int mode, int C, int K, const int* dil);
 bool resblock2_preferred(int mode, int C, int K, const int* dil);
 int resblock2_geo64(int mode);
diff --git a/tts-3_amd/csrc/hifigan.cpp b/tts-3_amd/csrc/hifigan.cpp
--- a/tts-3_amd/csrc/hifigan.cpp
+++ b/tts-3_amd/csrc/hifigan.cpp
@@ -102,6 +102,7 @@
   const char* sb = std::getenv("TTS_MI355X_SUBBATCH");
   n_lanes_ = sb ? std::max(1, std::min(std::atoi(sb), 8)) : 2;
   rb2_geo64_ = resblock2_geo64(mode);
+  geo64_wide_ = mrf_geo64_wide(mode);
   const char* bp = std::getenv("TTS_MI355X_BF16_PLANES");
   planes16_ = mode == MATH_BF16 && !(bp && bp[0] == '0') && cfg_.num_upsamples >= 1 &&
               cfg_.upsample_factors[0] % 8 == 0;
@@ -210,7 +211,7 @@
       const ConvTile t = conv_tile(u.mode, u.tile);
       const bool tile_ok = !t.WINO && t.CK % 16 == 0 && ch % t.CK == 0 && ch % t.BM == 0;
       ups_fused_[i] = tile_ok && resblock3_up_supported(mode, ch, cfg_.resblock_kernel_sizes[0],
-                                                        cfg_.resblock_dilation_sizes[0]);
+                                                        cfg_.resblock_dilation_sizes[0], geo64_wide_);
     }
   }
   const float* post_w = hw[wi]; wi += 1;
@@ -613,7 +614,7 @@
         const double bytes = 4.0 * B * L1.Cout * (double)len * (K + 1) + 4.0 * 6.0 * L1.Cout * L1.Cin * L1.K +
                              4.0 * Un.Cin * Un.Cout * 2 * Un.U;
         const std::string nm = "mrf_block_k" + std::to_string(L1.K) + "_c" + std::to_string(L1.Cout);
-        run(prof, s, nm.c_str(), flops, bytes, [&] { launch_resblock3(L1.mode, ra, B, L1.Cout, L1.K, s); });
+        run(prof, s, nm.c_str(), flops, bytes, [&] { launch_resblock3(L1.mode, ra, B, L1.Cout, L1.K, geo64_wide_, s); });
         std::swap(bufO, bufT0);
       } else if (cfg_.resblock_type == 1 && rb.fused3) {
         ResBlock3Args ra{};
@@ -630,7 +631,7 @@
                              4.0 * 6.0 * L1.Cout * L1.Cin * L1.K;
         const std::string nm = "mrf_block_k" + std::to_string(L1.K) + "_c" + std::to_string(L1.Cout);
         zorder();
-        run(prof, sj, nm.c_str(), flops, bytes, [&] { launch_resblock3(L1.mode, ra, B, L1.Cout, L1.K, sj); });
+        run(prof, sj, nm.c_str(), flops, bytes, [&] { launch_resblock3(L1.mode, ra, B, L1.Cout, L1.K, geo64_wide_, sj); });
         zdone();
       } else if (cfg_.resblock_type == 1 && rb.fused) {
         for (int m = 0; m < 3; ++m) {
@@ -670,7 +671,7 @@
           const std::string nm = std::string(post ? "mrf_pair_post_k" : "mrf_pair_k") + std::to_string(L1.K) +
                                  "_c" + std::to_string(L1.Cout);
           if (last) zorder();
-          run(prof, sj, nm.c_str(), flops, bytes, [&] { launch_resblock_pair(L1.mode, pa, B, L1.K, L1.Cout, sj); });
+          run(prof, sj, nm.c_str(), flops, bytes, [&] { launch_resblock_pair(L1.mode, pa, B, L1.K, L1.Cout, geo64_wide_, sj); });
           if (last) zdone();
         }
       } else if (cfg_.resblock_type == 1) {
diff --git a/tts-3_amd/csrc/hifigan.hpp b/tts-3_amd/csrc/hifigan.hpp
--- a/tts-3_amd/csrc/hifigan.hpp
+++ b/tts-3_amd/csrc/hifigan.hpp
@@ -103,6 +103,7 @@
   int device_;
   int hop_ = 1;
   int rb2_geo64_ = 0;
+  int geo64_wide_ = 0;
   bool post_fusion_ = true;
   bool planes16_ = false;
   std::vector<char> ups_fused_;
diff --git a/tts-3_amd/csrc/kernels_resblock.hip b/tts-3_amd/csrc/kernels_resblock.hip
--- a/tts-3_amd/csrc/kernels_resblock.hip
+++ b/tts-3_amd/csrc/kernels_resblock.hip
@@ -13,8 +13,12 @@
 constexpr int kPostK = 7;
 constexpr int kPostHalo = 3;
 
-template <class S, int K, int C, int PD, int GEO, bool ALLX = false, bool POST = false>
+template <class S, int K, int C, int PD, int GEO, bool ALLX = false, bool POST = false, bool SWZ = false>
 struct PairCfg {
+  static_assert(!SWZ || (GEO == 0 && C == 64 && S::NP == 2 && ALLX), "SWZ: GEO 0 at 64 channels, two-piece rows");
+  using ROWS = Res3Rows<S::NP, SWZ>;
+  static constexpr int PITCH = ROWS::PITCH;
+  static_assert(SWZ || PITCH == S::ROWB, "the padded layout is the scheme's own row");
   static constexpr int RP_W = (GEO == 0 || GEO == 4 || GEO == 5 || GEO == 7) ? 256 : (GEO == 1 ? 192 : 128);
   static constexpr int LEAD = (K - 1) / 2;
   static constexpr int RP_BN = RP_W - 2 * LEAD;
@@ -27,29 +31,32 @@
   static constexpr int NC = C / 16;
   static constexpr int HMAX = (K - 1) * 5;
   static constexpr int XROWS = RP_W + HMAX;
-  static constexpr int XSZB = XROWS * S::ROWB;
+  static constexpr int XSZB = XROWS * PITCH;
   static constexpr int TROWS = RP_W + 32;
-  static constexpr int TSZB = NC * TROWS * S::ROWB;
+  static constexpr int TSZB = NC * TROWS * PITCH;
   static constexpr int XBUFS = ALLX ? NC : 2;
   static constexpr int LDSB0 = (XBUFS * XSZB > TSZB ? XBUFS * XSZB : TSZB);
   static constexpr int ZTB = POST ? C * RP_BN * 4 : 0;
   static constexpr int LDSB = LDSB0 > ZTB ? LDSB0 : ZTB;
   static constexpr int STRIDE = POST ? RP_BN - 2 * kPostHalo : RP_BN;
   static constexpr int UPT = (XROWS * 4 + NT - 1) / NT;
+  static constexpr int LDS_TOTAL = LDSB + NW * 4 + 2 * C * 4 + (POST ? C * kPostK : 1) * 4;
+  static_assert(!SWZ || LDS_TOTAL <= 80 * 1024, "SWZ: two workgroups per CU");
   static_assert(TM >= 1 && TM * WM * 32 == C && TN * WN * 32 == RP_W, "geometry");
 };
 
 #ifndef PAIR_W_B1
 #define PAIR_W_B1 3
 #endif
-template <class S, int K, int C, int PD, int GEO, bool ALLX, bool POST = false, int PL = 0>
+template <class S, int K, int C, int PD, int GEO, bool ALLX, bool POST = false, int PL = 0, bool SWZ = false>
 __global__ __launch_bounds__((PairCfg<S, K, C, PD, GEO, ALLX, POST>::NT)) __attribute__((amdgpu_waves_per_eu(
-    C > 64 ? (GEO >= 5 ? 2 : 1) : (S::NP == 1 && PAIR_W_B1 > 0 ? PAIR_W_B1 : ((C == 32 || GEO == 2) && S::ROWB <= 80 ? 3 : 1)))))
+    SWZ ? 2 : C > 64 ? (GEO >= 5 ? 2 : 1) : (S::NP == 1 && PAIR_W_B1 > 0 ? PAIR_W_B1 : ((C == 32 || GEO == 2) && S::ROWB <= 80 ? 3 : 1)))))
 void resblock_pair_kernel(ResPairArgs pa) {
   constexpr bool XB = (PL & kPlaneXB16) != 0, YB = (PL & kPlaneYB16) != 0;
   using PX = PlaneT<XB>;
   using PY = PlaneT<YB>;
-  using P = PairCfg<S, K, C, PD, GEO, ALLX, POST>;
+  using P = PairCfg<S, K, C, PD, GEO, ALLX, POST, SWZ>;
+  using ROWS = typename P::ROWS;
   constexpr int RP_W = P::RP_W, RP_BN = P::RP_BN;
   constexpr int NP = S::NP;
   constexpr bool H3 = S::SCALED;
@@ -148,7 +155,8 @@
     const int ts = tx0 - a1.pad + r;
     const bool ok = r < XW && ts >= 0 && ts < T;
     uvoff[i] = ok ? (unsigned)(4 * q) * chb + (unsigned)ts * PX::ES : OOB_OFF;
-    ulds[i] = r < XW ? r * S::ROWB + 8 * quad_pos(q) : -1;
+    const int qp = quad_pos(q);
+    ulds[i] = r < XW ? ROWS::off(r, qp >> 1) + 8 * (qp & 1) : -1;
   }
   f32x4 xall[ALLX ? NC : 1][P::UPT];
   auto load_x = [&](int c) {
@@ -171,7 +179,10 @@
           v[j] = lrelu2(xreg[i][j], a1.in_slope);
           if (H3) v[j] *= xscale;
         }
-        split_store4<S>(xl + ulds[i], v[0], v[1], v[2], v[3]);
+        unsigned char* dst[NP];
+#pragma unroll
+        for (int p = 0; p < NP; ++p) dst[p] = xl + ROWS::piece(ulds[i], p);
+        split_store4<S>(dst, v[0], v[1], v[2], v[3]);
       }
     }
   };
@@ -214,9 +225,10 @@
   auto read_x = [&](const unsigned char* xl, int k, f32x4 (*dst)[NP]) {
 #pragma unroll
     for (int n = 0; n < TN; ++n) {
-      const unsigned char* p = xl + (xrow0 + n * 32 + k * d) * S::ROWB + 16 * half;
-#pragma unroll
-      for (int q = 0; q < NP; ++q) dst[n][q] = *reinterpret_cast<const f32x4*>(p + 32 * q);
+      const int o = ROWS::off(xrow0 + k * d, half);
+#pragma unroll
+      for (int q = 0; q < NP; ++q)
+        dst[n][q] = *reinterpret_cast<const f32x4*>(xl + ROWS::piece(o, q) + n * 32 * P::PITCH);
     }
   };
 
@@ -304,13 +316,18 @@
 #pragma unroll
       for (int n = 0; n < TN; ++n)
 #pragma unroll
-        for (int gl = 0; gl < 2; ++gl)
-          store_xt8<S>(smem + (((mrow0 + m * 32) / 16 + gl) * P::TROWS + xrow0 + n * 32) * S::ROWB + 16 * half,
-                       acc[m][n], 8 * gl, tscale);
-    constexpr int ZB = (P::TROWS - RP_W) * S::ROWB;
+        for (int gl = 0; gl < 2; ++gl) {
+          const int o = ROWS::off(xrow0, half);
+          unsigned char* dst[NP];
+#pragma unroll
+          for (int p = 0; p < NP; ++p)
+            dst[p] = smem + (((mrow0 + m * 32) / 16 + gl) * P::TROWS + n * 32) * P::PITCH + ROWS::piece(o, p);
+          store_xt8<S>(dst, acc[m][n], 8 * gl, tscale);
+        }
+    constexpr int ZB = (P::TROWS - RP_W) * P::PITCH;
     for (int e = tid * 16; e < NC * ZB; e += NT * 16) {
       const int g = e / ZB;
-      *reinterpret_cast<f32x4*>(smem + (g * P::TROWS + RP_W) * S::ROWB + (e - g * ZB)) = f32x4{};
+      *reinterpret_cast<f32x4*>(smem + (g * P::TROWS + RP_W) * P::PITCH + (e - g * ZB)) = f32x4{};
     }
     __syncthreads();
     const Conv1dArgs& a2 = pa.c2;
@@ -330,9 +347,10 @@
     auto read_t = [&](int g, int k, f32x4 (*dst)[NP]) {
 #pragma unroll
       for (int n = 0; n < TN; ++n) {
-        const unsigned char* p = smem + (g * P::TROWS + trow0 + n * 32 + k) * S::ROWB + 16 * half;
-#pragma unroll
-        for (int q = 0; q < NP; ++q) dst[n][q] = *reinterpret_cast<const f32x4*>(p + 32 * q);
+        const int o = ROWS::off(trow0 + k, half);
+#pragma unroll
+        for (int q = 0; q < NP; ++q)
+          dst[n][q] = *reinterpret_cast<const f32x4*>(smem + (g * P::TROWS + n * 32) * P::PITCH + ROWS::piece(o, q));
       }
     };
     read_t(0, 0, bcur);
@@ -373,22 +391,22 @@
 }
 
 namespace {
-template <class S, int K, int C, int GEO>
+template <class S, int K, int C, int GEO, bool SWZ = false>
 void launch_pair_t(const ResPairArgs& a, int B, hipStream_t s) {
   constexpr bool AX = C == 64 && GEO != 2;
   constexpr int PD = S::NP == 1 ? RES_PD_B1 : 2;
   auto go = [&](auto pl_tag) {
     constexpr int PL = decltype(pl_tag)::value;
     if (a.post_w) {
-      using P = PairCfg<S, K, C, PD, GEO, AX, true>;
+      using P = PairCfg<S, K, C, PD, GEO, AX, true, SWZ>;
       static_assert(P::RP_BN - 2 * kPostHalo <= 256, "one conv_post column per thread");
       dim3 grid(ceil_div(a.c1.Tout, P::STRIDE), 1, B);
-      hipLaunchKernelGGL((resblock_pair_kernel<S, K, C, PD, GEO, AX, true, PL>), grid, dim3(P::NT), 0, s, a);
+      hipLaunchKernelGGL((resblock_pair_kernel<S, K, C, PD, GEO, AX, true, PL, SWZ>), grid, dim3(P::NT), 0, s, a);
       return;
     }
-    using P = PairCfg<S, K, C, PD, GEO, AX>;
+    using P = PairCfg<S, K, C, PD, GEO, AX, false, SWZ>;
     dim3 grid(ceil_div(a.c1.Tout, P::RP_BN), 1, B);
-    hipLaunchKernelGGL((resblock_pair_kernel<S, K, C, PD, GEO, AX, false, PL>), grid, dim3(P::NT), 0, s, a);
+    hipLaunchKernelGGL((resblock_pair_kernel<S, K, C, PD, GEO, AX, false, PL, SWZ>), grid, dim3(P::NT), 0, s, a);
   };
   if (a.c1.planes != 0) {
     constexpr bool OK = std::is_same<S, SchemeB1>::value;
@@ -409,7 +427,7 @@
 }
 
 template <class S, int K>
-void launch_pair_k(const ResPairArgs& a, int B, int C, hipStream_t s) {
+void launch_pair_k(const ResPairArgs& a, int B, int C, int wide64, hipStream_t s) {
   if constexpr (S::NP == 1) {
     if (C == 128) {
       static const int geo = [] {
@@ -434,6 +452,12 @@
       return;
     }
   }
+  if constexpr (std::is_same<S, SchemeH3>::value) {
+    if (C == 64 && (wide64 & kWide64Pair) && pair_geo64() == 1 && a.c1.planes == 0) {
+      launch_pair_t<S, K, 64, 0, true>(a, B, s);
+      return;
+    }
+  }
   if (C == 32) launch_pair_t<S, K, 32, 0>(a, B, s);
   else if (C == 64 && pair_geo64() == 2 && S::ROWB <= 80) launch_pair_t<S, K, 64, 2>(a, B, s);
   else if (C == 64 && pair_geo64() == 4 && S::NP == 1) launch_pair_t<S, K, 64, 4>(a, B, s);
@@ -442,11 +466,11 @@
 }
 
 template <class S>
-void launch_pair_s(const ResPairArgs& a, int B, int K, int C, hipStream_t s) {
+void launch_pair_s(const ResPairArgs& a, int B, int K, int C, int wide64, hipStream_t s) {
   switch (K) {
-    case 3: launch_pair_k<S, 3>(a, B, C, s); break;
-    case 7: launch_pair_k<S, 7>(a, B, C, s); break;
-    case 11: launch_pair_k<S, 11>(a, B, C, s); break;
+    case 3: launch_pair_k<S, 3>(a, B, C, wide64, s); break;
+    case 7: launch_pair_k<S, 7>(a, B, C, wide64, s); break;
+    case 11: launch_pair_k<S, 11>(a, B, C, wide64, s); break;
     default: throw Error(3, "resblock pair: kernel size must be 3, 7 or 11");
   }
 }
@@ -473,7 +497,7 @@
   return resblock_pair_supported(mode, C, K, dil);
 }
 
-void launch_resblock_pair(int mode, const ResPairArgs& a, int B, int K, int C, hipStream_t s) {
+void launch_resblock_pair(int mode, const ResPairArgs& a, int B, int K, int C, int wide64, hipStream_t s) {
   TTS_REQUIRE(resblock_pair_supported(mode, C, K, a.c1.dil), 3, "resblock pair: unsupported configuration");
   TTS_REQUIRE(a.c1.Cin == C && a.c1.Cout == C && a.c2.Cin == C && a.c2.Cout == C && a.c1.Tin == a.c1.Tout &&
                   a.c2.Tout == a.c1.Tout && a.c1.rep_pad == 0 && a.c2.dil == 1,
@@ -484,9 +508,9 @@
   TTS_REQUIRE((int64_t)C * a.c1.Tout * 4 < (int64_t(1) << 31), 3, "resblock pair: plane exceeds 2 GiB");
   TTS_REQUIRE(!a.post_w || (a.c2.zmode == 3 && a.c2.res && a.c2.z && a.wav && !a.c2.mask), 1,
               "resblock pair: the fused conv_post needs the final MRF sum (zmode 3) with a residual");
-  if (mode == MATH_FP32_F16X3) launch_pair_s<SchemeH3>(a, B, K, C, s);
-  else if (mode == MATH_BF16) launch_pair_s<SchemeB1>(a, B, K, C, s);
-  else launch_pair_s<SchemeX6>(a, B, K, C, s);
+  if (mode == MATH_FP32_F16X3) launch_pair_s<SchemeH3>(a, B, K, C, wide64, s);
+  else if (mode == MATH_BF16) launch_pair_s<SchemeB1>(a, B, K, C, 0, s);
+  else launch_pair_s<SchemeX6>(a, B, K, C, 0, s);
   TTS_HIP_CHECK(hipGetLastError());
 }
 
@@ -504,8 +528,15 @@
   dim3 grid(ceil_div(a.T, P::RP_BN), 1, B);
   hipLaunchKernelGGL((resblock3_kernel<S, C, GEO, 3, 6, r3_xoff(3), r3_lead(3), 0, true>), grid, dim3(P::NT), 0, s, a);
 }
+template <class S, bool UP>
+void launch_res3_wide64(const ResBlock3Args& a, int B, hipStream_t s) {
+  using P = Res3Cfg<S, 64, 0, 3, 6, r3_xoff(3), r3_lead(3), UP, true>;
+  static_assert(P::RP_BN == 232, "kept columns [12, 244)");
+  dim3 grid(ceil_div(a.T, P::RP_BN), 1, B);
+  hipLaunchKernelGGL((resblock3_kernel<S, 64, 0, 3, 6, r3_xoff(3), r3_lead(3), 0, UP, true>), grid, dim3(P::NT), 0, s, a);
+}
 template <class S>
-void launch_res3_s(const ResBlock3Args& a, int B, int C, int K, hipStream_t s) {
+void launch_res3_s(const ResBlock3Args& a, int B, int C, int K, int wide64, hipStream_t s) {
   if (K == 7) {
     if (C == 32) launch_res3_t<S, 32, 0, 7>(a, B, s);
     else launch_res3_t<S, 64, 0, 7>(a, B, s);
@@ -515,6 +546,12 @@
     if (C == 32) launch_res3_t<S, 32, 0, 11>(a, B, s);
     else launch_res3_t<S, 64, 0, 11>(a, B, s);
     return;
+  }
+  if constexpr (std::is_same<S, SchemeH3>::value) {
+    if (C == 64 && (wide64 & kWide64Block) && a.planes == 0) {
+      launch_res3_wide64<S, false>(a, B, s);
+      return;
+    }
   }
   if (C == 32) launch_res3_t<S, 32, 0, 3>(a, B, s);
   else if (C == 128) {
@@ -543,9 +580,15 @@
   return lo <= r3_lead(K);
 }
 
-bool resblock3_up_supported(int mode, int C, int K, const int* dil) {
+int mrf_geo64_wide(int mode) {
+  if (mode != MATH_FP32_F16X3) return 0;
+  const char* e = std::getenv("TTS_MI355X_GEO64_WIDE");
+  return e && e[0] == '0' ? 0 : (kWide64Block | kWide64Pair);
+}
+
+bool resblock3_up_supported(int mode, int C, int K, const int* dil, int wide64) {
   if (mode != MATH_FP32_F16X3 || K != 3 || !(C == 64 || C == 128) || !resblock3_supported(mode, C, K, dil)) return false;
-  const int rp_w = 128;
+  const int rp_w = C == 64 && (wide64 & kWide64Block) ? 256 : 128;
   int lo = -r3_xoff(K), hi = rp_w + r3_xoff(K);
   for (int m = 0; m < 3; ++m) {
     lo = std::max(lo + dil[m], 0) + 1;
@@ -554,24 +597,25 @@
   return lo <= r3_lead(K) - 1 && hi >= rp_w - r3_lead(K) + 1;
 }
 
-void launch_resblock3(int mode, const ResBlock3Args& a, int B, int C, int K, hipStream_t s) {
+void launch_resblock3(int mode, const ResBlock3Args& a, int B, int C, int K, int wide64, hipStream_t s) {
   TTS_REQUIRE(resblock3_supported(mode, C, K, a.dil), 3, "resblock3: unsupported configuration");
   TTS_REQUIRE((int64_t)C * a.T * 4 < (int64_t(1) << 31), 3, "resblock3: plane exceeds 2 GiB");
   if (a.up_w) {
-    TTS_REQUIRE(resblock3_up_supported(mode, C, K, a.dil), 3, "resblock3: no upsampling tail for this configuration");
+    TTS_REQUIRE(resblock3_up_supported(mode, C, K, a.dil, wide64), 3, "resblock3: no upsampling tail for this configuration");
     TTS_REQUIRE(a.x && a.up_y && a.up_y != a.x && a.up_bias && a.planes == 0 && a.nzp >= 0 && a.nzp <= 2, 1,
                 "resblock3: bad arguments of the upsampling tail");
     for (int p = 0; p < a.nzp; ++p)
       TTS_REQUIRE(a.zp[p] && a.zp[p] != a.up_y, 1, "resblock3: a branch plane is missing or aliases the tail's output");
     if (C == 128) launch_res3_up_t<SchemeH3, 128, 4>(a, B, s);
+    else if (wide64 & kWide64Block) launch_res3_wide64<SchemeH3, true>(a, B, s);
     else launch_res3_up_t<SchemeH3, 64, 2>(a, B, s);
     TTS_HIP_CHECK(hipGetLastError());
     return;
   }
   TTS_REQUIRE(a.zmode >= 1 && a.zmode <= 3 && a.z && a.x && a.x != a.z, 1, "resblock3: bad arguments");
-  if (mode == MATH_FP32_F16X3) launch_res3_s<SchemeH3>(a, B, C, K, s);
-  else if (mode == MATH_BF16) launch_res3_s<SchemeB1>(a, B, C, K, s);
-  else launch_res3_s<SchemeX6>(a, B, C, K, s);
+  if (mode == MATH_FP32_F16X3) launch_res3_s<SchemeH3>(a, B, C, K, wide64, s);
+  else if (mode == MATH_BF16) launch_res3_s<SchemeB1>(a, B, C, K, 0, s);
+  else launch_res3_s<SchemeX6>(a, B, C, K, 0, s);
   TTS_HIP_CHECK(hipGetLastError());
 }
 
diff --git a/tts-3_amd/csrc/resblock_block.hpp b/tts-3_amd/csrc/resblock_block.hpp
--- a/tts-3_amd/csrc/resblock_block.hpp
+++ b/tts-3_amd/csrc/resblock_block.hpp
@@ -22,8 +22,12 @@
 constexpr int r3_lead(int K) { return R3_LEAD * ((K - 1) / 2); }
 constexpr int rb2_halo(int K) { return K == 3 ? 4 : (K == 5 ? 12 : (K == 7 ? 9 : 15)); }
 
-template <class S, int C, int GEO, int K = 3, int NCV = 6, int XO = R3_XOFF, int LEAD = R3_LEAD, bool UP = false>
+template <class S, int C, int GEO, int K = 3, int NCV = 6, int XO = R3_XOFF, int LEAD = R3_LEAD, bool UP = false,
+          bool SW = false>
 struct Res3Cfg {
+  static_assert(!SW || (GEO == 0 && S::NP == 2), "SW: GEO 0's tile, two-piece rows");
+  static constexpr bool SWZ = (GEO == 4 || SW) && S::NP == 2;
+  static constexpr bool W64 = GEO == 4 || SW;
   static constexpr int RP_W = GEO == 0 ? 256 : (GEO == 1 ? 192 : 128);
   static constexpr int RP_BN = RP_W - 2 * LEAD;
   static constexpr int NW = GEO == 3 ? 8 : 4;
@@ -34,11 +38,11 @@
   static constexpr int TN = RP_W / 32 / WN;
   static constexpr int NC = C / 16;
   static constexpr int PR = RP_W + 2 * XO;
-  using ROWS = Res3Rows<S::NP, GEO == 4 && S::NP == 2>;
-  static_assert(GEO == 4 || ROWS::PITCH == S::ROWB, "the padded layout is the scheme's own row");
+  using ROWS = Res3Rows<S::NP, SWZ>;
+  static_assert(SWZ || ROWS::PITCH == S::ROWB, "the padded layout is the scheme's own row");
   static constexpr int LDSB = NC * PR * ROWS::PITCH;
   static constexpr int LDS_TOTAL = LDSB + 2 * NW * 4 + (NCV + UP) * C * 4;
-  static_assert(GEO != 4 || LDS_TOTAL <= 80 * 1024, "GEO 4: two workgroups per CU");
+  static_assert(!W64 || LDS_TOTAL <= 80 * 1024, "GEO 4 / SW: two workgroups per CU");
   static_assert(TM >= 1 && TM * WM * 32 == C && TN * WN * 32 == RP_W, "geometry");
 };
 
@@ -48,15 +52,15 @@
 #ifndef RB3_W64
 #define RB3_W64 2
 #endif
-template <class S, int C, int GEO, int K, int NCV, int XO, int LEAD, int PL = 0, bool UP = false>
+template <class S, int C, int GEO, int K, int NCV, int XO, int LEAD, int PL = 0, bool UP = false, bool SW = false>
 __global__ __launch_bounds__((Res3Cfg<S, C, GEO, K, NCV, XO, LEAD>::NT))
 __attribute__((amdgpu_waves_per_eu(S::NP == 1 && RB3_W_B1 > 0 ? RB3_W_B1
-                                                                : (C == 64 && GEO == 2 ? RB3_W64 : (C == 32 || GEO >= 3 ? 2 : 1)))))
+                                                                : (C == 64 && GEO == 2 ? RB3_W64 : (C == 32 || GEO >= 3 || SW ? 2 : 1)))))
 void resblock3_kernel(ResBlock3Args a) {
   constexpr bool XB = (PL & kPlaneXB16) != 0, YB = (PL & kPlaneYB16) != 0;
   using PX = PlaneT<XB>;
   using PY = PlaneT<YB>;
-  using P = Res3Cfg<S, C, GEO, K, NCV, XO, LEAD, UP>;
+  using P = Res3Cfg<S, C, GEO, K, NCV, XO, LEAD, UP, SW>;
   using ROWS = typename P::ROWS;
   static_assert(NCV == 6 || NCV == 2, "ResBlock1 (6 convs) or ResBlock2 (2 convs)");
   static_assert(!UP || (NCV == 6 && S::SCALED && PL == 0), "the upsampling tail: ResBlock1, f16x3, fp32 planes");
@@ -89,7 +93,7 @@
     if constexpr (XB) return PX::ld(rx, off, soff);
     else return bload_x<decltype(pol_tag)::value>(rx, off, soff);
   };
-  constexpr bool SOFF = GEO == 4;
+  constexpr bool SOFF = P::W64;
 
   int ex = H3 ? amax_exp(a.amax_in, b) : 0;
   f32x16 xr[TM][TN];
@@ -391,7 +395,7 @@
       for (int n = 0; n < TN; ++n) {
         const int col = xcol0 + n * 32;
         const int t = tx0 + col;
-        const bool tok = t >= 0 && t < T;
+        const bool tok = t >= 0 && t < T && col >= lo && col < hi;
         const unsigned vlane = tok ? (unsigned)(4 * half) * chb + (unsigned)t * 4u : OOB_OFF;
         __builtin_amdgcn_sched_barrier(0);
         float pv[2][16];
@@ -517,7 +521,7 @@
       else if constexpr (UP) final_up(2 * it + 1);
       else final_to_z(2 * it + 1);
     };
-    if constexpr (GEO == 4 || UP) {
+    if constexpr (P::W64 || UP) {
 #pragma unroll 1
       for (int it = 0; it < 2; ++it) iteration(it, std::integral_constant<int, 1>{});
       iteration(2, std::integral_constant<int, 2>{});
diff --git a/tts-3_amd/tests_native/geo64_layout_check.cpp b/tts-3_amd/tests_native/geo64_layout_check.cpp
--- /dev/null
+++ b/tts-3_amd/tests_native/geo64_layout_check.cpp
@@ -0,0 +1,207 @@
+#include <algorithm>
+#include <cstdio>
+#include <vector>
+
+#include "common.hpp"
+#include "res3_layout.hpp"
+
+using namespace tts;
+
+static int failures = 0;
+#define CHECK(cond, ...)                          \
+  do {                                            \
+    if (!(cond)) {                                \
+      if (failures < 20) {                        \
+        std::fprintf(stderr, "FAIL: " __VA_ARGS__); \
+        std::fprintf(stderr, "\n");               \
+      }                                           \
+      ++failures;                                 \
+    }                                             \
+  } while (0)
+
+using R = Res3Rows<2, true>;
+constexpr int NP = 2, NC = 4, RP_W = 256, NT = 256, PITCH = R::PITCH;
+static long n_reads = 0, n_stores = 0;
+
+static int worst(const std::vector<int>& addr, const std::vector<int>& lanes, int dw, int banks) {
+  std::vector<std::vector<int>> on(banks);
+  for (int l : lanes) {
+    if (addr[l] < 0) continue;
+    for (int j = 0; j < dw; ++j) {
+      const int d = addr[l] / 4 + j;
+      auto& v = on[d % banks];
+      if (std::find(v.begin(), v.end(), d) == v.end()) v.push_back(d);
+    }
+  }
+  size_t w = 0;
+  for (const auto& v : on) w = std::max(w, v.size());
+  return (int)w;
+}
+
+static std::vector<std::vector<int>> read128_groups() {
+  const int a[2][16] = {{0, 1, 2, 3, 12, 13, 14, 15, 20, 21, 22, 23, 24, 25, 26, 27},
+                        {4, 5, 6, 7, 8, 9, 10, 11, 16, 17, 18, 19, 28, 29, 30, 31}};
+  std::vector<std::vector<int>> g;
+  for (int h = 0; h < 2; ++h)
+    for (int s = 0; s < 2; ++s) {
+      std::vector<int> v;
+      for (int i = 0; i < 16; ++i) v.push_back(a[s][i] + 32 * h);
+      g.push_back(v);
+    }
+  return g;
+}
+static std::vector<std::vector<int>> contiguous_groups(int n) {
+  std::vector<std::vector<int>> g;
+  for (int l0 = 0; l0 < 64; l0 += n) {
+    std::vector<int> v;
+    for (int i = 0; i < n; ++i) v.push_back(l0 + i);
+    g.push_back(v);
+  }
+  return g;
+}
+
+static const std::vector<std::vector<int>> RG = read128_groups(), W8 = contiguous_groups(8), W16 = contiguous_groups(16);
+
+static void expect_read(const std::vector<int>& addr, const char* what, int a, int b, int c, int d) {
+  for (const auto& grp : RG)
+    CHECK(worst(addr, grp, 4, 64) == 1, "%s: ds_read_b128 conflict (%d %d %d %d)", what, a, b, c, d);
+  ++n_reads;
+}
+static void expect_store(const std::vector<int>& addr, bool b128, const char* what, int a, int b, int c, int d) {
+  for (const auto& grp : b128 ? W8 : W16)
+    CHECK(worst(addr, grp, b128 ? 4 : 2, 32) <= 2, "%s: %s conflict above 2-way (%d %d %d %d)", what,
+          b128 ? "ds_write_b128" : "ds_write_b64", a, b, c, d);
+  ++n_stores;
+}
+
+static void check_pair(int K) {
+  const int XROWS = RP_W + (K - 1) * 5, XSZB = XROWS * PITCH, TROWS = RP_W + 32;
+  const int LDSB = std::max(NC * XSZB, NC * TROWS * PITCH);
+  const int UPT = (XROWS * 4 + NT - 1) / NT;
+  CHECK(LDSB + 4 * 4 + 2 * 64 * 4 + 64 * 7 * 4 <= 80 * 1024, "pair k%d: LDS %d B does not fit twice", K, LDSB);
+  std::vector<int> addr(64);
+  for (int d : {1, 3, 5}) {
+    const int XW = RP_W + (K - 1) * d;
+    for (int c = 0; c < NC; ++c)
+      for (int i = 0; i < UPT; ++i)
+        for (int wave = 0; wave < 4; ++wave)
+          for (int p = 0; p < NP; ++p) {
+            for (int lane = 0; lane < 64; ++lane) {
+              const int u = wave * 64 + lane + i * NT;
+              const int q = quad_pos((u >> 3) & 3), r = (u >> 5) * 8 + (u & 7), qp = quad_pos(q);
+              const int ulds = r < XW ? R::off(r, qp >> 1) + 8 * (qp & 1) : -1;
+              addr[lane] = ulds < 0 ? -1 : c * XSZB + R::piece(ulds, p);
+              if (ulds >= 0) {
+                CHECK(addr[lane] >= c * XSZB + r * PITCH && addr[lane] + 8 <= c * XSZB + (r + 1) * PITCH,
+                      "pair k%d: staging store leaves row %d of buffer %d", K, r, c);
+                CHECK(addr[lane] == c * XSZB + R::off(r, (qp >> 1) + 2 * p) + 8 * (qp & 1), "pair k%d: staging piece()", K);
+              }
+            }
+            expect_store(addr, false, "pair staging", K, d, c, i);
+          }
+    for (int c = 0; c < NC; ++c)
+      for (int wn = 0; wn < 4; ++wn)
+        for (int n = 0; n < 2; ++n)
+          for (int k = 0; k < K; ++k)
+            for (int q = 0; q < NP; ++q) {
+              for (int lane = 0; lane < 64; ++lane) {
+                const int half = lane >> 5, row = wn * 64 + (lane & 31) + k * d;
+                addr[lane] = c * XSZB + R::piece(R::off(row, half), q) + n * 32 * PITCH;
+                CHECK(row + n * 32 < XW, "pair k%d: tap read of an unstaged row %d", K, row + n * 32);
+                CHECK(addr[lane] == c * XSZB + R::off(row + n * 32, half + 2 * q), "pair k%d: read and store disagree, row %d",
+                      K, row + n * 32);
+              }
+              expect_read(addr, "pair tap", K, d, c, k);
+            }
+  }
+  for (int g = 0; g < NC; ++g)
+    for (int wn = 0; wn < 4; ++wn)
+      for (int n = 0; n < 2; ++n) {
+        for (int p = 0; p < NP; ++p) {
+          for (int lane = 0; lane < 64; ++lane) {
+            const int half = lane >> 5, row = wn * 64 + (lane & 31);
+            addr[lane] = (g * TROWS + n * 32) * PITCH + R::piece(R::off(row, half), p);
+            CHECK(addr[lane] == g * TROWS * PITCH + R::off(row + n * 32, half + 2 * p), "pair k%d: store_xt8 unit map", K);
+            CHECK(addr[lane] + 16 <= LDSB, "pair k%d: store_xt8 leaves the LDS array", K);
+          }
+          expect_store(addr, true, "pair store_xt8", K, g, wn, n);
+        }
+        for (int k = 0; k <= 10; ++k)
+          for (int q = 0; q < NP; ++q) {
+            for (int lane = 0; lane < 64; ++lane) {
+              const int half = lane >> 5, row = wn * 64 + (lane & 31) + k;
+              addr[lane] = (g * TROWS + n * 32) * PITCH + R::piece(R::off(row, half), q);
+              CHECK(row + n * 32 < TROWS, "pair k%d: phase-2 read past the zero rows", K);
+              CHECK(addr[lane] == g * TROWS * PITCH + R::off(row + n * 32, half + 2 * q), "pair k%d: phase-2 unit map", K);
+              CHECK(addr[lane] + 16 <= LDSB, "pair k%d: phase-2 read leaves the LDS array", K);
+            }
+            expect_read(addr, "pair phase 2", K, g, wn, k);
+          }
+      }
+}
+
+static void check_block() {
+  constexpr int XO = 5, HK = 1, PR = RP_W + 2 * XO, LDSB = NC * PR * PITCH;
+  static_assert(LDSB + 2 * 4 * 4 + 7 * 64 * 4 <= 80 * 1024, "the block fits twice");
+  std::vector<int> addr(64);
+  struct Tap { int roff, kstep, ntaps; };
+  std::vector<Tap> taps;
+  for (int d : {1, 3, 5}) taps.push_back({XO - HK * d, d, 3});
+  taps.push_back({0, 1, 3});
+  taps.push_back({XO - 1, 1, 2});
+  for (const Tap& t : taps)
+    for (int g = 0; g < NC; ++g)
+      for (int wn = 0; wn < 4; ++wn)
+        for (int n = 0; n < 2; ++n)
+          for (int k = 0; k < t.ntaps; ++k)
+            for (int q = 0; q < NP; ++q) {
+              for (int lane = 0; lane < 64; ++lane) {
+                const int half = lane >> 5, row = g * PR + wn * 64 + (lane & 31) + t.roff + k * t.kstep;
+                addr[lane] = R::piece(R::off(row, half), q) + n * 32 * PITCH;
+                CHECK(row + n * 32 >= g * PR && row + n * 32 < (g + 1) * PR, "block: read row outside group %d", g);
+                CHECK(addr[lane] == R::off(row + n * 32, half + 2 * q), "block: read unit map, row %d", row + n * 32);
+              }
+              expect_read(addr, "block tap", t.roff, t.kstep, g, k);
+            }
+  for (int roff : {XO, HK})
+    for (int g = 0; g < NC; ++g)
+      for (int wn = 0; wn < 4; ++wn)
+        for (int n = 0; n < 2; ++n)
+          for (int p = 0; p < NP; ++p) {
+            for (int lane = 0; lane < 64; ++lane) {
+              const int half = lane >> 5, row = g * PR + wn * 64 + (lane & 31) + roff;
+              addr[lane] = R::piece(R::off(row, half), p) + n * 32 * PITCH;
+              CHECK(addr[lane] == R::off(row + n * 32, half + 2 * p), "block: store_pieces unit map");
+              CHECK(addr[lane] + 16 <= LDSB, "block: store_pieces leaves the LDS array");
+            }
+            expect_store(addr, true, "block store_pieces", roff, g, wn, n);
+          }
+  for (int g = 0; g < NC; ++g)
+    for (int u0 = 0; u0 < ((PR * 4 + NT - 1) / NT) * NT; u0 += 64)
+      for (int p = 0; p < NP; ++p) {
+        for (int lane = 0; lane < 64; ++lane) {
+          const int u = u0 + lane;
+          const int q = quad_pos((u >> 3) & 3), r = (u >> 5) * 8 + (u & 7), qp = quad_pos(q);
+          addr[lane] = r < PR ? R::off(g * PR + r, (qp >> 1) + 2 * p) + 8 * (qp & 1) : -1;
+        }
+        expect_store(addr, false, "block prologue", g, u0, p, 0);
+      }
+}
+
+int main() {
+  static_assert(R::PITCH == 64 && R::SWIZZLED, "the swizzled two-piece row");
+  for (int K : {3, 7, 11}) check_pair(K);
+  check_block();
+  {
+    std::vector<int> addr(64);
+    for (int lane = 0; lane < 64; ++lane) addr[lane] = (lane & 31) * 64 + 16 * (lane >> 5);
+    CHECK(worst(addr, RG[0], 4, 64) == 4, "the replay does not see the 4-way conflict of plain 64-byte rows");
+  }
+  if (failures) {
+    std::fprintf(stderr, "%d layout check(s) failed\n", failures);
+    return 1;
+  }
+  std::printf("geo64_layout_check: %ld read and %ld store instructions replayed: reads conflict-free, stores at most 2-way\n",
+              n_reads, n_stores);
+  return 0;
+}
```

Result: faster. 172.1 million samples/s (median of 6 runs) (+1.2%).
